# eps696/aphantasia

Hardware: NVIDIA H100
Metric: optimization steps/sec @1280x720 FFT, 200 samples, ViT-B/32 (higher is better)
Workload: dtype bf16

## Files before the change

aphantasia_b200/_lib.py:

```python
import ctypes as C
import os

_HERE = os.path.dirname(os.path.abspath(__file__))
LIB_PATH = os.path.join(_HERE, 'libaphb200.so')

_lib = None

c_f32p = C.c_void_p
_SIGS = {
    'aph_version': (C.c_int, []),
    'aph_last_error': (C.c_char_p, []),
    'aph_launch_count': (C.c_int64, []),
    'aph_fft_plan_create': (C.c_int, [C.POINTER(C.c_void_p), C.c_int, C.c_int]),
    'aph_fft_plan_destroy': (C.c_int, [C.c_void_p]),
    'aph_synth_fft_fwd': (C.c_int, [C.c_void_p, c_f32p, c_f32p, c_f32p, C.c_int, C.c_float, C.c_void_p, C.c_int,
                                    c_f32p, C.c_void_p, c_f32p, C.c_void_p]),
    'aph_synth_fft_bwd': (C.c_int, [C.c_void_p, c_f32p, c_f32p, c_f32p, C.c_void_p, c_f32p, C.c_float, C.c_void_p, C.c_int,
                                    c_f32p, C.c_void_p]),
    'aph_dwt_plan_create': (C.c_int, [C.POINTER(C.c_void_p), C.c_int, C.c_int, C.c_void_p, C.c_void_p, C.c_int]),
    'aph_dwt_plan_destroy': (C.c_int, [C.c_void_p]),
    'aph_dwt_plan_levels': (C.c_int, [C.c_void_p, C.POINTER(C.c_int), C.c_void_p, C.c_void_p]),
    'aph_synth_dwt_fwd': (C.c_int, [C.c_void_p, C.c_void_p, C.c_void_p, C.c_float, C.c_void_p, C.c_int, c_f32p, C.c_void_p, c_f32p, C.c_void_p]),
    'aph_synth_dwt_bwd': (C.c_int, [C.c_void_p, c_f32p, c_f32p, c_f32p, C.c_void_p, C.c_void_p, C.c_float, C.c_void_p, C.c_int, C.c_void_p, C.c_void_p]),
    'aph_pixel_fwd': (C.c_int, [c_f32p, C.c_int64, C.c_float, C.c_int, C.c_void_p, C.c_int, C.c_void_p, c_f32p, C.c_void_p]),
    'aph_pixel_bwd': (C.c_int, [c_f32p, c_f32p, c_f32p, C.c_void_p, C.c_int64, C.c_float, C.c_int, C.c_void_p, C.c_int, c_f32p, C.c_void_p]),
    'aph_valid_rgb_fwd': (C.c_int, [c_f32p, C.c_int64, C.c_void_p, c_f32p, C.c_void_p]),
    'aph_valid_rgb_bwd': (C.c_int, [c_f32p, c_f32p, C.c_int64, C.c_void_p, c_f32p, C.c_void_p]),
    'aph_sample_fwd': (C.c_int, [c_f32p, C.c_int, C.c_int, C.c_int, C.c_int, c_f32p, C.c_int, C.c_int, C.c_int, c_f32p, C.c_void_p]),
    'aph_sample_fwd_patches': (C.c_int, [c_f32p, C.c_int, C.c_int, C.c_int, C.c_int, c_f32p, C.c_int, C.c_int, C.c_int, c_f32p, C.c_void_p, C.c_int,
                                         C.POINTER(C.c_int), C.c_void_p]),
    'aph_sample_bwd': (C.c_int, [c_f32p, C.c_int, C.c_int, C.c_int, C.c_int, c_f32p, C.c_int, C.c_int, C.c_int, c_f32p, C.c_void_p]),
    'aph_sample_bwd_scaled': (C.c_int, [c_f32p, C.c_int, C.c_int, C.c_int, C.c_int, c_f32p, C.c_int, C.c_int, C.c_int, C.c_float, c_f32p, C.c_void_p]),
    'aph_rng_crop_tables': (C.c_int, [C.c_void_p, C.c_int64, C.c_void_p, C.POINTER(C.c_int32), C.c_void_p, C.c_void_p, C.c_void_p, C.c_int,
                                      C.c_int, C.c_int, C.c_int, C.c_int, C.c_int, C.c_int, C.c_float, C.c_int, C.c_void_p]),
    'aph_vit_create': (C.c_int, [C.POINTER(C.c_void_p), C.c_void_p]),
    'aph_vit_destroy': (C.c_int, [C.c_void_p]),
    'aph_vit_load_tensor': (C.c_int, [C.c_void_p, C.c_char_p, c_f32p, C.c_int64, C.c_void_p]),
    'aph_vit_finalize': (C.c_int, [C.c_void_p]),
    'aph_vit_fwd': (C.c_int, [C.c_void_p, c_f32p, C.c_int, c_f32p, C.c_int, C.c_void_p]),
    'aph_vit_patch_operand': (C.c_int, [C.c_void_p, C.c_int, C.POINTER(C.c_void_p), C.POINTER(C.c_int), C.POINTER(C.c_int)]),
    'aph_vit_fwd_prepatched': (C.c_int, [C.c_void_p, C.c_int, c_f32p, C.c_int, C.c_void_p]),
    'aph_vit_bwd': (C.c_int, [C.c_void_p, c_f32p, C.c_int, c_f32p, C.c_void_p]),
    'aph_vit_bytes': (C.c_int64, [C.c_void_p]),
    'aph_text_create': (C.c_int, [C.POINTER(C.c_void_p), C.c_void_p]),
    'aph_text_destroy': (C.c_int, [C.c_void_p]),
    'aph_text_load_tensor': (C.c_int, [C.c_void_p, C.c_char_p, c_f32p, C.c_int64, C.c_void_p]),
    'aph_text_finalize': (C.c_int, [C.c_void_p]),
    'aph_text_fwd': (C.c_int, [C.c_void_p, C.c_void_p, C.c_int, c_f32p, C.c_void_p]),
    'aph_text_bytes': (C.c_int64, [C.c_void_p]),
    'aph_gemm_bf16_tn': (C.c_int, [C.c_void_p, C.c_void_p, c_f32p, C.c_int, C.c_int, C.c_int, C.c_void_p]),
    'aph_gemm_epi_test': (C.c_int, [C.c_void_p, C.c_void_p, C.c_int, C.c_int, C.c_int, c_f32p, c_f32p, C.c_void_p, C.c_int, c_f32p, C.c_void_p, C.c_void_p,
                                    C.c_int, C.c_int, C.c_void_p]),
    'aph_gemm_variant_launches': (C.c_int64, [C.c_int, C.c_int]),
    'aph_prof_gemm': (C.c_int, [C.c_int, C.POINTER(C.c_double), C.POINTER(C.c_double), C.POINTER(C.c_int)]),
    'aph_sim_fwd': (C.c_int, [c_f32p, C.c_int, c_f32p, C.c_int, C.c_int, C.c_int, c_f32p, c_f32p, c_f32p, C.c_void_p]),
    'aph_derivat_fwd': (C.c_int, [c_f32p, C.c_int, C.c_int, C.c_int, C.c_void_p, c_f32p, C.c_void_p]),
    'aph_derivat_bwd': (C.c_int, [c_f32p, C.c_int, C.c_int, C.c_int, c_f32p, c_f32p, C.c_void_p]),
    'aph_head_fwd': (C.c_int, [c_f32p, C.c_int, C.c_int, c_f32p, c_f32p, c_f32p, C.c_void_p]),
    'aph_head_bwd': (C.c_int, [c_f32p, c_f32p, C.c_int, C.c_int, c_f32p, C.c_void_p]),
    'aph_synth_fft_bwd_adam': (C.c_int, [C.c_void_p, c_f32p, c_f32p, c_f32p, C.c_void_p, c_f32p, C.c_float, C.c_void_p, C.c_int,
                                         c_f32p, c_f32p, c_f32p, c_f32p, C.c_float, C.c_float, C.c_float, C.c_float, C.c_int, C.c_void_p]),
    'aph_allreduce_sym': (C.c_int, [C.c_uint64, C.c_void_p, C.c_uint64, C.c_int, C.c_int, C.c_int64, C.c_void_p, C.c_void_p]),
    'aph_adam_step': (C.c_int, [c_f32p, c_f32p, c_f32p, c_f32p, C.c_int64, C.c_float, C.c_float, C.c_float, C.c_float, C.c_int, C.c_void_p]),
}
EXPORTS = tuple(_SIGS)


class VitConfig(C.Structure):
    _fields_ = [(n, C.c_int32) for n in ('patch', 'width', 'layers', 'heads', 'out_dim', 'res', 'max_batch', 'reserved')]


class TextConfig(C.Structure):
    _fields_ = [(n, C.c_int32) for n in ('width', 'layers', 'heads', 'out_dim', 'context', 'vocab', 'max_batch', 'reserved')]


def lib():
    global _lib
    if _lib is None:
        if not os.path.isfile(LIB_PATH):
            raise RuntimeError('aphantasia_b200: %s not built. Run `python -c "import __graft_entry__ as g; g.build()"` '
                               '(or `make -C aphantasia_b200/csrc`). There is no CPU fallback.' % LIB_PATH)
        l = C.CDLL(LIB_PATH)
        for name, (res, args) in _SIGS.items():
            f = getattr(l, name)
            f.restype, f.argtypes = res, args
        _lib = l
    return _lib


def check(rc, what):
    if rc != 0:
        raise RuntimeError('%s failed (rc=%d): %s' % (what, rc, lib().aph_last_error().decode('utf-8', 'replace')))


def stream_ptr():
    import torch
    return torch.cuda.current_stream().cuda_stream


def require_cuda(t, name):
    import torch
    if not (isinstance(t, torch.Tensor) and t.is_cuda):
        raise RuntimeError('aphantasia_b200: %s must be a CUDA tensor; this implementation has no CPU path' % name)
```

aphantasia_b200/csrc/tc_gemm.cuh:

```cuda
#pragma once
#include "aph_common.cuh"
#include <cuda.h>

namespace aph {

typedef __nv_bfloat16 bf16;

struct GemmEpi {
  const float* bias = nullptr;
  const float* resid = nullptr;
  const bf16* gelu_in = nullptr;
  float* out_f32 = nullptr;
  bf16* out_bf16 = nullptr;
  bf16* out_pre = nullptr;
  int act = 0;
  int unpatch_p = 0;
  int unpatch_g = 0;
};

struct GemmShape { int M, N, K; };

constexpr int GEMM_BM = 128;
constexpr int GEMM_BK = 64;
constexpr int GEMM_UK = 16;
constexpr int GEMM_THREADS = 3 * 128;

enum : int {
  EPI_F32 = 0,
  EPI_BF16 = 1,
  EPI_BIAS_BF16 = 2,
  EPI_BIAS_GELU = 3,
  EPI_BIAS_RESID = 4,
  EPI_GELUGRAD_BF16 = 5,
  EPI_UNPATCH = 6,
  EPI_KINDS = 7
};

__device__ __forceinline__ uint32_t smem_u32(const void* p) { return (uint32_t)__cvta_generic_to_shared(p); }

__device__ __forceinline__ void mbar_init(uint64_t* bar, uint32_t count) {
  asm volatile("mbarrier.init.shared::cta.b64 [%0], %1;" ::"r"(smem_u32(bar)), "r"(count));
}
__device__ __forceinline__ void mbar_expect_tx(uint64_t* bar, uint32_t bytes) {
  asm volatile("mbarrier.arrive.expect_tx.shared::cta.b64 _, [%0], %1;" ::"r"(smem_u32(bar)), "r"(bytes) : "memory");
}
__device__ __forceinline__ void mbar_arrive(uint64_t* bar) {
  asm volatile("mbarrier.arrive.shared::cta.b64 _, [%0];" ::"r"(smem_u32(bar)) : "memory");
}
__device__ __forceinline__ void mbar_wait(uint64_t* bar, uint32_t parity) {
  uint32_t done;
  do {
    asm volatile(
        "{\n\t.reg .pred p;\n\t"
        "mbarrier.try_wait.parity.shared::cta.b64 p, [%1], %2;\n\t"
        "selp.u32 %0, 1, 0, p;\n\t}"
        : "=r"(done) : "r"(smem_u32(bar)), "r"(parity) : "memory");
  } while (!done);
}
__device__ __forceinline__ void fence_barrier_init() { asm volatile("fence.mbarrier_init.release.cluster;" ::: "memory"); }

__device__ __forceinline__ void tma_prefetch_desc(const CUtensorMap* m) {
  asm volatile("prefetch.tensormap [%0];" ::"l"(reinterpret_cast<uint64_t>(m)) : "memory");
}
__device__ __forceinline__ void tma_load_2d(void* dst, const CUtensorMap* m, uint64_t* bar, int x, int y) {
  asm volatile("cp.async.bulk.tensor.2d.shared::cluster.global.mbarrier::complete_tx::bytes [%0], [%1, {%3, %4}], [%2];"
               ::"r"(smem_u32(dst)), "l"(reinterpret_cast<uint64_t>(m)), "r"(smem_u32(bar)), "r"(x), "r"(y) : "memory");
}
__device__ __forceinline__ void tma_load_3d(uint32_t dst_saddr, const CUtensorMap* m, uint64_t* bar, int x, int y, int z) {
  asm volatile("cp.async.bulk.tensor.3d.shared::cluster.global.mbarrier::complete_tx::bytes [%0], [%1, {%3, %4, %5}], [%2];"
               ::"r"(dst_saddr), "l"(reinterpret_cast<uint64_t>(m)), "r"(smem_u32(bar)), "r"(x), "r"(y), "r"(z) : "memory");
}
__device__ __forceinline__ void tma_load_2d_hint(void* dst, const CUtensorMap* m, uint64_t* bar, int x, int y, uint64_t policy) {
  asm volatile("cp.async.bulk.tensor.2d.shared::cluster.global.mbarrier::complete_tx::bytes.L2::cache_hint [%0], [%1, {%3, %4}], [%2], %5;"
               ::"r"(smem_u32(dst)), "l"(reinterpret_cast<uint64_t>(m)), "r"(smem_u32(bar)), "r"(x), "r"(y), "l"(policy) : "memory");
}
__device__ __forceinline__ uint64_t l2_policy_evict_last() {
  uint64_t p;
  asm volatile("createpolicy.fractional.L2::evict_last.b64 %0, 1.0;" : "=l"(p));
  return p;
}

__device__ __forceinline__ uint64_t make_smem_desc(uint32_t saddr) {
  uint64_t d = 0;
  d |= (uint64_t)((saddr & 0x3FFFF) >> 4);
  d |= (uint64_t)1 << 16;
  d |= (uint64_t)(1024 >> 4) << 32;
  d |= (uint64_t)1 << 62;
  return d;
}
__device__ __forceinline__ void wgmma_fence() { asm volatile("wgmma.fence.sync.aligned;" ::: "memory"); }
__device__ __forceinline__ void wgmma_commit() { asm volatile("wgmma.commit_group.sync.aligned;" ::: "memory"); }
template <int N> __device__ __forceinline__ void wgmma_wait() { asm volatile("wgmma.wait_group.sync.aligned %0;" ::"n"(N) : "memory"); }
template <int R> __device__ __forceinline__ void setmaxnreg_inc() { asm volatile("setmaxnreg.inc.sync.aligned.u32 %0;" ::"n"(R)); }
template <int R> __device__ __forceinline__ void setmaxnreg_dec() { asm volatile("setmaxnreg.dec.sync.aligned.u32 %0;" ::"n"(R)); }

template <int BN> struct Wgmma;
#define APH_WG_REGS8(o) "+f"(d[o]), "+f"(d[o + 1]), "+f"(d[o + 2]), "+f"(d[o + 3]), "+f"(d[o + 4]), "+f"(d[o + 5]), "+f"(d[o + 6]), "+f"(d[o + 7])
template <> struct Wgmma<128> {
  static __device__ __forceinline__ void mma(float (&d)[64], uint64_t da, uint64_t db, int acc) {
    asm volatile(
        "{\n\t.reg .pred p;\n\tsetp.ne.b32 p, %66, 0;\n\t"
        "wgmma.mma_async.sync.aligned.m64n128k16.f32.bf16.bf16 "
        "{%0, %1, %2, %3, %4, %5, %6, %7, %8, %9, %10, %11, %12, %13, %14, %15, %16, %17, %18, %19, %20, %21, %22, %23, "
        "%24, %25, %26, %27, %28, %29, %30, %31, %32, %33, %34, %35, %36, %37, %38, %39, %40, %41, %42, %43, %44, %45, %46, %47, "
        "%48, %49, %50, %51, %52, %53, %54, %55, %56, %57, %58, %59, %60, %61, %62, %63}, %64, %65, p, 1, 1, 0, 0;\n\t}"
        : APH_WG_REGS8(0), APH_WG_REGS8(8), APH_WG_REGS8(16), APH_WG_REGS8(24), APH_WG_REGS8(32), APH_WG_REGS8(40), APH_WG_REGS8(48), APH_WG_REGS8(56)
        : "l"(da), "l"(db), "r"(acc));
  }
};
template <> struct Wgmma<256> {
  static __device__ __forceinline__ void mma(float (&d)[128], uint64_t da, uint64_t db, int acc) {
    asm volatile(
        "{\n\t.reg .pred p;\n\tsetp.ne.b32 p, %130, 0;\n\t"
        "wgmma.mma_async.sync.aligned.m64n256k16.f32.bf16.bf16 "
        "{%0, %1, %2, %3, %4, %5, %6, %7, %8, %9, %10, %11, %12, %13, %14, %15, %16, %17, %18, %19, %20, %21, %22, %23, "
        "%24, %25, %26, %27, %28, %29, %30, %31, %32, %33, %34, %35, %36, %37, %38, %39, %40, %41, %42, %43, %44, %45, %46, %47, "
        "%48, %49, %50, %51, %52, %53, %54, %55, %56, %57, %58, %59, %60, %61, %62, %63, %64, %65, %66, %67, %68, %69, %70, %71, "
        "%72, %73, %74, %75, %76, %77, %78, %79, %80, %81, %82, %83, %84, %85, %86, %87, %88, %89, %90, %91, %92, %93, %94, %95, "
        "%96, %97, %98, %99, %100, %101, %102, %103, %104, %105, %106, %107, %108, %109, %110, %111, %112, %113, %114, %115, "
        "%116, %117, %118, %119, %120, %121, %122, %123, %124, %125, %126, %127}, %128, %129, p, 1, 1, 0, 0;\n\t}"
        : APH_WG_REGS8(0), APH_WG_REGS8(8), APH_WG_REGS8(16), APH_WG_REGS8(24), APH_WG_REGS8(32), APH_WG_REGS8(40), APH_WG_REGS8(48), APH_WG_REGS8(56),
          APH_WG_REGS8(64), APH_WG_REGS8(72), APH_WG_REGS8(80), APH_WG_REGS8(88), APH_WG_REGS8(96), APH_WG_REGS8(104), APH_WG_REGS8(112), APH_WG_REGS8(120)
        : "l"(da), "l"(db), "r"(acc));
  }
};
#undef APH_WG_REGS8

__device__ __forceinline__ float sigmoid1702(float x) {
  float t;
  asm("tanh.approx.f32 %0, %1;" : "=f"(t) : "f"(0.851f * x));
  return fmaf(0.5f, t, 0.5f);
}
__device__ __forceinline__ float quickgelu(float x) { return x * sigmoid1702(x); }
__device__ __forceinline__ float quickgelu_grad(float x) {
  const float s = sigmoid1702(x);
  return s * (1.f + 1.702f * x * (1.f - s));
}
__device__ __forceinline__ uint32_t pack_bf16(float lo, float hi) {
  __nv_bfloat162 v = __floats2bfloat162_rn(lo, hi);
  return *reinterpret_cast<uint32_t*>(&v);
}

template <int BN>
struct GemmCfg {
  static constexpr int A_BYTES = GEMM_BM * GEMM_BK * 2;
  static constexpr int B_BYTES = BN * GEMM_BK * 2;
  static constexpr int STAGE_BYTES = A_BYTES + B_BYTES;
  static constexpr int STAGES = (BN == 256) ? 4 : 6;
  static constexpr int BAR_OFFSET = STAGES * STAGE_BYTES;
  static constexpr int SMEM = BAR_OFFSET + 2 * STAGES * 8 + 1024;
};

__device__ __forceinline__ void consumer_bar_sync(int id) { asm volatile("bar.sync %0, 256;" ::"r"(id) : "memory"); }
__device__ __forceinline__ void consumer_bar_arrive(int id) { asm volatile("bar.arrive %0, 256;" ::"r"(id) : "memory"); }

template <int EPI>
constexpr bool epi_bf16_out() { return EPI == EPI_BF16 || EPI == EPI_BIAS_BF16 || EPI == EPI_BIAS_GELU || EPI == EPI_GELUGRAD_BF16; }

template <int EPI>
__device__ __forceinline__ void epi_store2(const GemmEpi& epi, int N, int row, int col, float v0, float v1, float2 bb) {
  const size_t off = (size_t)row * N + col;
  if (EPI == EPI_F32) {
    *reinterpret_cast<float2*>(epi.out_f32 + off) = make_float2(v0, v1);
  } else if (EPI == EPI_BIAS_RESID) {
    const float2 r = __ldg(reinterpret_cast<const float2*>(epi.resid + off));
    *reinterpret_cast<float2*>(epi.out_f32 + off) = make_float2(v0 + bb.x + r.x, v1 + bb.y + r.y);
  } else {
    const int p = epi.unpatch_p, g = epi.unpatch_g, R = p * g;
    const int ch = col / (p * p), rem = col - ch * p * p, py = rem / p, px = rem - py * p;
    const int s = row / (g * g), pr = row - s * g * g, gy = pr / g, gx = pr - gy * g;
    *reinterpret_cast<float2*>(epi.out_f32 + (((size_t)s * 3 + ch) * R + gy * p + py) * R + gx * p + px) = make_float2(v0, v1);
  }
}

__device__ __forceinline__ void st_global_16(void* p, const uint32_t (&w)[4]) {
  asm volatile("st.global.v4.b32 [%0], {%1, %2, %3, %4};" ::"l"(p), "r"(w[0]), "r"(w[1]), "r"(w[2]), "r"(w[3]) : "memory");
}

__device__ __forceinline__ void quad_transpose(uint32_t (&w)[4], int q) {
  const bool b0 = q & 1, b1 = q & 2;
#pragma unroll
  for (int p = 0; p < 2; ++p) {
    const uint32_t r = __shfl_xor_sync(0xffffffffu, b0 ? w[2 * p] : w[2 * p + 1], 1);
    if (b0) w[2 * p] = r; else w[2 * p + 1] = r;
  }
#pragma unroll
  for (int p = 0; p < 2; ++p) {
    const uint32_t r = __shfl_xor_sync(0xffffffffu, b1 ? w[p] : w[p + 2], 2);
    if (b1) w[p] = r; else w[p + 2] = r;
  }
}

template <int EPI>
__device__ __forceinline__ void epi_store_bf16x32(const GemmEpi& epi, int N, int row, bool valid, int col0, int q, const float* v,
                                                  const float2* bb) {
  const size_t off = (size_t)row * N + col0 + 8 * q;
  uint32_t w[4], w2[4];
  if constexpr (EPI == EPI_GELUGRAD_BF16) {
    uint4 g = make_uint4(0u, 0u, 0u, 0u);
    if (valid) g = __ldg(reinterpret_cast<const uint4*>(epi.gelu_in + off));
    w2[0] = g.x; w2[1] = g.y; w2[2] = g.z; w2[3] = g.w;
    quad_transpose(w2, q);
  }
#pragma unroll
  for (int t = 0; t < 4; ++t) {
    float v0 = v[2 * t], v1 = v[2 * t + 1];
    if (EPI == EPI_BF16) {
      w[t] = pack_bf16(v0, v1);
    } else if (EPI == EPI_BIAS_BF16) {
      w[t] = pack_bf16(v0 + bb[t].x, v1 + bb[t].y);
    } else if (EPI == EPI_BIAS_GELU) {
      v0 += bb[t].x; v1 += bb[t].y;
      w2[t] = pack_bf16(v0, v1);
      w[t] = pack_bf16(quickgelu(v0), quickgelu(v1));
    } else {
      const float2 h = __bfloat1622float2(*reinterpret_cast<const __nv_bfloat162*>(&w2[t]));
      w[t] = pack_bf16(v0 * quickgelu_grad(h.x), v1 * quickgelu_grad(h.y));
    }
  }
  quad_transpose(w, q);
  if (valid) st_global_16(epi.out_bf16 + off, w);
  if constexpr (EPI == EPI_BIAS_GELU) {
    quad_transpose(w2, q);
    if (valid) st_global_16(epi.out_pre + off, w2);
  }
}

template <int BN, bool PINGPONG, int EPI>
__global__ void __launch_bounds__(GEMM_THREADS, 1)
k_gemm_bf16_tn(const __grid_constant__ CUtensorMap map_a, const __grid_constant__ CUtensorMap map_b, GemmShape shp, GemmEpi epi) {
  static_assert(BN == 128 || !PINGPONG, "the ping-pong schedule runs 128 x 128 tiles");
  using L = GemmCfg<BN>;
  constexpr int STAGES = L::STAGES;
  constexpr int MMAS = PINGPONG ? 2 : 1;
  constexpr bool HAS_BIAS = (EPI == EPI_BIAS_BF16 || EPI == EPI_BIAS_GELU || EPI == EPI_BIAS_RESID);
  pdl_trigger();
  extern __shared__ uint8_t smem_raw[];
  uint8_t* smem = reinterpret_cast<uint8_t*>((reinterpret_cast<uintptr_t>(smem_raw) + 1023) & ~(uintptr_t)1023);
  uint64_t* full_bar = reinterpret_cast<uint64_t*>(smem + L::BAR_OFFSET);
  uint64_t* empty_bar = full_bar + STAGES;

  const int wg = threadIdx.x >> 7, tid = threadIdx.x & 127;
  const int m_tiles = (shp.M + GEMM_BM - 1) / GEMM_BM, n_tiles = shp.N / BN;
  const int num_tiles = m_tiles * n_tiles, k_blocks = shp.K / GEMM_BK;

  if (threadIdx.x == 0) {
    tma_prefetch_desc(&map_a); tma_prefetch_desc(&map_b);
    for (int i = 0; i < STAGES; ++i) { mbar_init(&full_bar[i], 1); mbar_init(&empty_bar[i], PINGPONG ? 1 : 2); }
    fence_barrier_init();
  }
  __syncthreads();
  pdl_wait();

  if (wg == 0) {
    setmaxnreg_dec<40>();
    if (tid == 0) {
      const uint64_t pol_b = l2_policy_evict_last();
      uint32_t it = 0;
      for (int tile = blockIdx.x; tile < num_tiles; tile += gridDim.x) {
        const int m_blk = tile / n_tiles, n_blk = tile - m_blk * n_tiles;
        for (int kb = 0; kb < k_blocks; ++kb, ++it) {
          const uint32_t s = it % STAGES, ph = (it / STAGES) & 1;
          mbar_wait(&empty_bar[s], ph ^ 1);
          uint8_t* sa = smem + s * L::STAGE_BYTES;
          mbar_expect_tx(&full_bar[s], L::STAGE_BYTES);
          tma_load_2d(sa, &map_a, &full_bar[s], kb * GEMM_BK, m_blk * GEMM_BM);
          tma_load_2d_hint(sa + L::A_BYTES, &map_b, &full_bar[s], kb * GEMM_BK, n_blk * BN, pol_b);
        }
      }
    }
  } else {
    setmaxnreg_inc<232>();
    const int c = wg - 1, warp = tid >> 5, lane = tid & 31;
    const int row_in_tile = (PINGPONG ? 0 : 64 * c) + 16 * warp + (lane >> 2), col_in_tile = 2 * (lane & 3);
    uint32_t it = PINGPONG ? c * k_blocks : 0;
    const int tile_step = (PINGPONG ? 2 : 1) * gridDim.x;
    for (int tile = blockIdx.x + (PINGPONG ? c * gridDim.x : 0); tile / n_tiles * GEMM_BM < shp.M; tile += tile_step) {
      if (PINGPONG && tile != (int)blockIdx.x) consumer_bar_sync(1 + c);
      float d[MMAS][BN / 2];
#pragma unroll
      for (int h = 0; h < MMAS; ++h)
#pragma unroll
        for (int r = 0; r < BN / 2; ++r) d[h][r] = 0.f;
      for (int kb = 0; kb < k_blocks; ++kb, ++it) {
        const uint32_t s = it % STAGES, ph = (it / STAGES) & 1;
        mbar_wait(&full_bar[s], ph);
        const uint64_t ds = make_smem_desc(smem_u32(smem + s * L::STAGE_BYTES));
        wgmma_fence();
#pragma unroll
        for (int k = 0; k < GEMM_BK / GEMM_UK; ++k)
#pragma unroll
          for (int h = 0; h < MMAS; ++h)
            Wgmma<BN>::mma(d[h], ds + (uint64_t)((PINGPONG ? h : c) * 512 + 2 * k), ds + (uint64_t)(L::A_BYTES / 16 + 2 * k), (kb | k) != 0);
        wgmma_commit();
        wgmma_wait<1>();
        if (kb > 0 && tid == 0) mbar_arrive(&empty_bar[(it - 1) % STAGES]);
      }
      if (PINGPONG && (tile + (int)gridDim.x) / n_tiles * GEMM_BM < shp.M) consumer_bar_arrive(1 + (c ^ 1));
      wgmma_wait<0>();
      if (tid == 0) mbar_arrive(&empty_bar[(it - 1) % STAGES]);
      if (PINGPONG) it += k_blocks;
      const int m_blk = tile / n_tiles, n_blk = tile - m_blk * n_tiles;
#pragma unroll
      for (int h = 0; h < MMAS; ++h) {
        const int row0 = m_blk * GEMM_BM + 64 * h + row_in_tile, row1 = row0 + 8;
        if constexpr (epi_bf16_out<EPI>()) {
#pragma unroll
          for (int j0 = 0; j0 < BN / 8; j0 += 4) {
            const int col0 = n_blk * BN + 8 * j0;
            float2 bb[4];
            float v0[8], v1[8];
#pragma unroll
            for (int t = 0; t < 4; ++t) {
              bb[t] = HAS_BIAS ? __ldg(reinterpret_cast<const float2*>(epi.bias + col0 + 8 * t + col_in_tile)) : make_float2(0.f, 0.f);
              v0[2 * t] = d[h][4 * (j0 + t)]; v0[2 * t + 1] = d[h][4 * (j0 + t) + 1];
              v1[2 * t] = d[h][4 * (j0 + t) + 2]; v1[2 * t + 1] = d[h][4 * (j0 + t) + 3];
            }
            epi_store_bf16x32<EPI>(epi, shp.N, row0, row0 < shp.M, col0, lane & 3, v0, bb);
            epi_store_bf16x32<EPI>(epi, shp.N, row1, row1 < shp.M, col0, lane & 3, v1, bb);
          }
        } else {
#pragma unroll
          for (int j = 0; j < BN / 8; ++j) {
            const int col = n_blk * BN + 8 * j + col_in_tile;
            const float2 bb = HAS_BIAS ? __ldg(reinterpret_cast<const float2*>(epi.bias + col)) : make_float2(0.f, 0.f);
            if (row0 < shp.M) epi_store2<EPI>(epi, shp.N, row0, col, d[h][4 * j], d[h][4 * j + 1], bb);
            if (row1 < shp.M) epi_store2<EPI>(epi, shp.N, row1, col, d[h][4 * j + 2], d[h][4 * j + 3], bb);
          }
        }
      }
    }
  }
}

int make_tmap_bf16(CUtensorMap* out, const void* base, int rows, int K, int box_rows);
int make_tmap_bf16_tokens(CUtensorMap* out, const void* base, int cols, int T, int S, int box_rows);
int launch_gemm(const void* A, const void* B, GemmShape shp, const GemmEpi& epi, cudaStream_t st);

}
```

aphantasia_b200/csrc/vit.cu:

```cuda
#include "vit_ops.cuh"
#include "vit_attn_tc.cuh"
#include <stdlib.h>
#include <string>
#include <vector>
#include <map>
#include <string.h>

namespace aph {

struct LayerW {
  float *ln1_w = nullptr, *ln1_b = nullptr, *ln2_w = nullptr, *ln2_b = nullptr;
  float *b_qkv = nullptr, *b_o = nullptr, *b_fc = nullptr, *b_proj = nullptr;
  bf16 *w_qkv = nullptr, *w_qkv_t = nullptr;
  bf16 *w_o = nullptr, *w_o_t = nullptr;
  bf16 *w_fc = nullptr, *w_fc_t = nullptr;
  bf16 *w_proj = nullptr, *w_proj_t = nullptr;
};

struct VitImpl {
  aph_vit_config cfg;
  int g, T, D, Kp;
  int64_t bytes = 0;
  std::vector<void*> allocs;
  bf16 *w_conv = nullptr, *w_conv_t = nullptr;
  float *cls = nullptr, *pos = nullptr, *lnpre_w = nullptr, *lnpre_b = nullptr, *lnpost_w = nullptr, *lnpost_b = nullptr;
  bf16 *w_out = nullptr, *w_out_t = nullptr;
  std::vector<LayerW> L;
  std::map<std::string, bool> loaded;
  bool finalized = false;
  bf16* patches = nullptr;
  float* tok = nullptr;
  float* e = nullptr;
  std::vector<float*> xs;
  bf16* ln_out = nullptr;
  std::vector<bf16*> qkv;
  bf16* attn_out = nullptr;
  std::vector<bf16*> h_pre;
  bf16* h_act = nullptr;
  float *st_mean = nullptr, *st_rstd = nullptr;
  bf16* cls_ln = nullptr;
  float* emb_int = nullptr;
  bf16* d_emb = nullptr;
  float* d_cls = nullptr;
  float* dx = nullptr;
  bf16* dx_bf = nullptr;
  bf16* dh = nullptr;
  bf16* d_ln = nullptr;
  bf16* d_attn = nullptr;
  bf16* d_qkv = nullptr;
  bf16* d_tok = nullptr;
  int last_S = -1;
  struct GraphEntry { const void* in; const void* out; int S; int flag; cudaGraphExec_t exec; unsigned long long stamp; int nodes; };
  std::vector<GraphEntry> fwd_graphs, bwd_graphs;
  std::map<int, int> warm_fwd, warm_bwd;
  unsigned long long stamp = 0;
  int graph_misses = 0;
};

bool gemm_profiling_on();

static bool graphs_enabled() {
  static int v = -1;
  if (v < 0) { const char* e = getenv("APH_VIT_GRAPH"); v = (e && e[0] == '0') ? 0 : 1; }
  return v == 1 && !gemm_profiling_on();
}

template <typename Body>
static int run_cached(std::vector<VitImpl::GraphEntry>& cache, std::map<int, int>& warm, unsigned long long& stamp, int& misses,
                      const void* in, const void* out, int S, int flag, cudaStream_t& st, Body body) {
  if (!graphs_enabled() || misses > 6) return body();
  for (auto& g : cache)
    if (g.in == in && g.out == out && g.S == S && g.flag == flag) {
      g.stamp = ++stamp;
      misses = 0;
      APH_CUDA_OK(cudaGraphLaunch(g.exec, st));
      count_launch(g.nodes);
      return 0;
    }
  if (!warm[S]) { warm[S] = 1; return body(); }
  static cudaStream_t cap = nullptr;
  if (!cap) APH_CUDA_OK(cudaStreamCreateWithFlags(&cap, cudaStreamNonBlocking));
  cudaStream_t user = st;
  st = cap;
  if (cudaStreamBeginCapture(cap, cudaStreamCaptureModeThreadLocal) != cudaSuccess) { cudaGetLastError(); st = user; return body(); }
  const int rc = body();
  cudaGraph_t graph = nullptr;
  const cudaError_t ce = cudaStreamEndCapture(cap, &graph);
  st = user;
  if (rc != 0 || ce != cudaSuccess || graph == nullptr) {
    if (graph) cudaGraphDestroy(graph);
    cudaGetLastError();
    if (rc != 0) return rc;
    return body();
  }
  size_t nodes = 0;
  cudaGraphGetNodes(graph, nullptr, &nodes);
  g_launches.fetch_sub((long long)nodes, std::memory_order_relaxed);
  cudaGraphExec_t exec = nullptr;
  if (cudaGraphInstantiate(&exec, graph, 0) != cudaSuccess) { cudaGraphDestroy(graph); cudaGetLastError(); return body(); }
  cudaGraphDestroy(graph);
  if (cache.size() >= 4) {
    size_t lru = 0;
    for (size_t i = 1; i < cache.size(); ++i) if (cache[i].stamp < cache[lru].stamp) lru = i;
    cudaGraphExecDestroy(cache[lru].exec);
    cache.erase(cache.begin() + lru);
  }
  ++misses;
  cache.push_back({in, out, S, flag, exec, ++stamp, (int)nodes});
  APH_CUDA_OK(cudaGraphLaunch(exec, st));
  count_launch((int)nodes);
  return 0;
}

template <typename Tp>
static int dev_alloc(VitImpl* v, Tp** p, size_t count) {
  void* q = nullptr;
  APH_CUDA_OK(cudaMalloc(&q, count * sizeof(Tp)));
  v->allocs.push_back(q);
  v->bytes += (int64_t)(count * sizeof(Tp));
  *p = reinterpret_cast<Tp*>(q);
  return 0;
}

__global__ void __launch_bounds__(256) k_pack_weight(const float* __restrict__ in, bf16* __restrict__ out, int rows, int cols, int transpose) {
  const size_t n = (size_t)rows * cols;
  for (size_t i = blockIdx.x * (size_t)blockDim.x + threadIdx.x; i < n; i += (size_t)gridDim.x * blockDim.x) {
    const int r = (int)(i / cols), c = (int)(i - (size_t)r * cols);
    const bf16 v = __float2bfloat16_rn(in[i]);
    if (transpose) out[(size_t)c * rows + r] = v; else out[i] = v;
  }
}

int pack(const float* src, bf16* dst, int rows, int cols, int transpose, cudaStream_t st) {
  const size_t n = (size_t)rows * cols;
  const int blocks = (int)std::min<size_t>((n + 255) / 256, (size_t)num_sms() * 16);
  k_pack_weight<<<blocks, 256, 0, st>>>(src, dst, rows, cols, transpose);
  APH_LAUNCH_OK();
  return 0;
}

int copy_f32(const float* src, float* dst, size_t n, cudaStream_t st) {
  APH_CUDA_OK(cudaMemcpyAsync(dst, src, n * sizeof(float), cudaMemcpyDeviceToDevice, st));
  return 0;
}

static inline int rows_grid(int rows) { return (rows * 32 + 255) / 256; }

static bool attn_simt() {
  static int v = -1;
  if (v < 0) { const char* e = getenv("APH_ATTN_SIMT"); v = (e && e[0] == '1') ? 1 : 0; }
  return v == 1;
}

}

using namespace aph;

extern "C" int aph_vit_create(aph_vit** out, const aph_vit_config* cfg) {
  APH_REQUIRE(out && cfg, "aph_vit_create: null argument");
  APH_REQUIRE(cfg->width % 128 == 0 && (cfg->width / 128 == 1 || cfg->width / 128 == 2 || cfg->width / 128 == 6 || cfg->width / 128 == 8),
              "aph_vit_create: width %d unsupported (128, 256, 768, 1024)", cfg->width);
  APH_REQUIRE(cfg->heads * 64 == cfg->width, "aph_vit_create: head dim must be 64 (width %d, heads %d)", cfg->width, cfg->heads);
  APH_REQUIRE(cfg->res % cfg->patch == 0 && cfg->patch % 8 == 0, "aph_vit_create: res %d / patch %d", cfg->res, cfg->patch);
  APH_REQUIRE(cfg->out_dim % 128 == 0 && cfg->max_batch > 0 && cfg->layers > 0, "aph_vit_create: out_dim %d must be a multiple of 128", cfg->out_dim);
  VitImpl* v = new VitImpl();
  v->cfg = *cfg;
  v->g = cfg->res / cfg->patch; v->T = v->g * v->g + 1; v->D = cfg->width; v->Kp = 3 * cfg->patch * cfg->patch;
  APH_REQUIRE(v->T <= 256 && v->Kp % 128 == 0, "aph_vit_create: T=%d (max 256) Kp=%d", v->T, v->Kp);
  const int D = v->D, T = v->T, S = cfg->max_batch, Ly = cfg->layers, O = cfg->out_dim;
  const size_t M = (size_t)S * T, Mp = (size_t)S * v->g * v->g;
  int e = 0;
  e |= dev_alloc(v, &v->w_conv, (size_t)D * v->Kp); e |= dev_alloc(v, &v->w_conv_t, (size_t)D * v->Kp);
  e |= dev_alloc(v, &v->cls, D); e |= dev_alloc(v, &v->pos, (size_t)T * D);
  e |= dev_alloc(v, &v->lnpre_w, D); e |= dev_alloc(v, &v->lnpre_b, D); e |= dev_alloc(v, &v->lnpost_w, D); e |= dev_alloc(v, &v->lnpost_b, D);
  e |= dev_alloc(v, &v->w_out, (size_t)D * O); e |= dev_alloc(v, &v->w_out_t, (size_t)D * O);
  v->L.resize(Ly);
  for (auto& l : v->L) {
    e |= dev_alloc(v, &l.ln1_w, D); e |= dev_alloc(v, &l.ln1_b, D); e |= dev_alloc(v, &l.ln2_w, D); e |= dev_alloc(v, &l.ln2_b, D);
    e |= dev_alloc(v, &l.b_qkv, 3 * D); e |= dev_alloc(v, &l.b_o, D); e |= dev_alloc(v, &l.b_fc, 4 * D); e |= dev_alloc(v, &l.b_proj, D);
    e |= dev_alloc(v, &l.w_qkv, (size_t)3 * D * D); e |= dev_alloc(v, &l.w_qkv_t, (size_t)3 * D * D);
    e |= dev_alloc(v, &l.w_o, (size_t)D * D); e |= dev_alloc(v, &l.w_o_t, (size_t)D * D);
    e |= dev_alloc(v, &l.w_fc, (size_t)4 * D * D); e |= dev_alloc(v, &l.w_fc_t, (size_t)4 * D * D);
    e |= dev_alloc(v, &l.w_proj, (size_t)4 * D * D); e |= dev_alloc(v, &l.w_proj_t, (size_t)4 * D * D);
  }
  e |= dev_alloc(v, &v->patches, Mp * v->Kp); e |= dev_alloc(v, &v->tok, Mp * D); e |= dev_alloc(v, &v->e, M * D);
  v->xs.resize(2 * Ly + 1); for (auto& x : v->xs) e |= dev_alloc(v, &x, M * D);
  e |= dev_alloc(v, &v->ln_out, M * D); e |= dev_alloc(v, &v->attn_out, M * D); e |= dev_alloc(v, &v->h_act, M * 4 * D);
  v->qkv.resize(Ly); v->h_pre.resize(Ly);
  for (int i = 0; i < Ly; ++i) { e |= dev_alloc(v, &v->qkv[i], M * 3 * D); e |= dev_alloc(v, &v->h_pre[i], M * 4 * D); }
  e |= dev_alloc(v, &v->st_mean, (size_t)(2 * Ly + 2) * M); e |= dev_alloc(v, &v->st_rstd, (size_t)(2 * Ly + 2) * M);
  e |= dev_alloc(v, &v->cls_ln, (size_t)S * D); e |= dev_alloc(v, &v->emb_int, (size_t)S * O);
  e |= dev_alloc(v, &v->d_emb, (size_t)S * O); e |= dev_alloc(v, &v->d_cls, (size_t)S * D);
  e |= dev_alloc(v, &v->dx, M * D); e |= dev_alloc(v, &v->dx_bf, M * D); e |= dev_alloc(v, &v->dh, M * 4 * D);
  e |= dev_alloc(v, &v->d_ln, M * D); e |= dev_alloc(v, &v->d_attn, M * D); e |= dev_alloc(v, &v->d_qkv, M * 3 * D);
  e |= dev_alloc(v, &v->d_tok, Mp * D);
  if (e) { aph_vit_destroy(reinterpret_cast<aph_vit*>(v)); return 1; }
  APH_CUDA_OK(cudaFuncSetAttribute(k_attn_fwd, cudaFuncAttributeMaxDynamicSharedMemorySize, (int)attn_fwd_smem(T)));
  APH_CUDA_OK(cudaFuncSetAttribute(k_attn_bwd, cudaFuncAttributeMaxDynamicSharedMemorySize, (int)attn_bwd_smem(T)));
  *out = reinterpret_cast<aph_vit*>(v);
  return 0;
}

extern "C" int aph_vit_destroy(aph_vit* vit) {
  if (!vit) return 0;
  VitImpl* v = reinterpret_cast<VitImpl*>(vit);
  for (auto& g : v->fwd_graphs) cudaGraphExecDestroy(g.exec);
  for (auto& g : v->bwd_graphs) cudaGraphExecDestroy(g.exec);
  for (void* p : v->allocs) cudaFree(p);
  delete v;
  return 0;
}

extern "C" int64_t aph_vit_bytes(const aph_vit* vit) { return vit ? reinterpret_cast<const VitImpl*>(vit)->bytes : 0; }

extern "C" int aph_vit_load_tensor(aph_vit* vit, const char* key, const float* data, int64_t numel, void* stream) {
  APH_REQUIRE(vit && key && data, "aph_vit_load_tensor: null argument");
  VitImpl* v = reinterpret_cast<VitImpl*>(vit);
  cudaStream_t st = (cudaStream_t)stream;
  const int D = v->D, O = v->cfg.out_dim;
  std::string k(key);
  if (k.rfind("visual.", 0) == 0) k = k.substr(7);
  auto need = [&](int64_t n) -> int { APH_REQUIRE(numel == n, "aph_vit_load_tensor(%s): expected %lld elements, got %lld", key, (long long)n, (long long)numel); return 0; };
  int e = 0;
  if (k == "conv1.weight") { if ((e = need((int64_t)D * v->Kp))) return e; e = pack(data, v->w_conv, D, v->Kp, 0, st) | pack(data, v->w_conv_t, D, v->Kp, 1, st); }
  else if (k == "class_embedding") { if ((e = need(D))) return e; e = copy_f32(data, v->cls, D, st); }
  else if (k == "positional_embedding") { if ((e = need((int64_t)v->T * D))) return e; e = copy_f32(data, v->pos, (size_t)v->T * D, st); }
  else if (k == "ln_pre.weight") { if ((e = need(D))) return e; e = copy_f32(data, v->lnpre_w, D, st); }
  else if (k == "ln_pre.bias") { if ((e = need(D))) return e; e = copy_f32(data, v->lnpre_b, D, st); }
  else if (k == "ln_post.weight") { if ((e = need(D))) return e; e = copy_f32(data, v->lnpost_w, D, st); }
  else if (k == "ln_post.bias") { if ((e = need(D))) return e; e = copy_f32(data, v->lnpost_b, D, st); }
  else if (k == "proj") {
    if ((e = need((int64_t)D * O))) return e;
    e = pack(data, v->w_out, D, O, 1, st) | pack(data, v->w_out_t, D, O, 0, st);
  } else if (k.rfind("transformer.resblocks.", 0) == 0) {
    const char* rest = k.c_str() + strlen("transformer.resblocks.");
    char* endp = nullptr;
    const long li = strtol(rest, &endp, 10);
    APH_REQUIRE(endp && *endp == '.' && li >= 0 && li < v->cfg.layers, "aph_vit_load_tensor: bad layer index in %s", key);
    LayerW& l = v->L[li];
    const std::string f(endp + 1);
    if (f == "ln_1.weight") { if ((e = need(D))) return e; e = copy_f32(data, l.ln1_w, D, st); }
    else if (f == "ln_1.bias") { if ((e = need(D))) return e; e = copy_f32(data, l.ln1_b, D, st); }
    else if (f == "ln_2.weight") { if ((e = need(D))) return e; e = copy_f32(data, l.ln2_w, D, st); }
    else if (f == "ln_2.bias") { if ((e = need(D))) return e; e = copy_f32(data, l.ln2_b, D, st); }
    else if (f == "attn.in_proj_weight") { if ((e = need((int64_t)3 * D * D))) return e; e = pack(data, l.w_qkv, 3 * D, D, 0, st) | pack(data, l.w_qkv_t, 3 * D, D, 1, st); }
    else if (f == "attn.in_proj_bias") { if ((e = need(3 * D))) return e; e = copy_f32(data, l.b_qkv, 3 * D, st); }
    else if (f == "attn.out_proj.weight") { if ((e = need((int64_t)D * D))) return e; e = pack(data, l.w_o, D, D, 0, st) | pack(data, l.w_o_t, D, D, 1, st); }
    else if (f == "attn.out_proj.bias") { if ((e = need(D))) return e; e = copy_f32(data, l.b_o, D, st); }
    else if (f == "mlp.c_fc.weight") { if ((e = need((int64_t)4 * D * D))) return e; e = pack(data, l.w_fc, 4 * D, D, 0, st) | pack(data, l.w_fc_t, 4 * D, D, 1, st); }
    else if (f == "mlp.c_fc.bias") { if ((e = need(4 * D))) return e; e = copy_f32(data, l.b_fc, 4 * D, st); }
    else if (f == "mlp.c_proj.weight") { if ((e = need((int64_t)4 * D * D))) return e; e = pack(data, l.w_proj, D, 4 * D, 0, st) | pack(data, l.w_proj_t, D, 4 * D, 1, st); }
    else if (f == "mlp.c_proj.bias") { if ((e = need(D))) return e; e = copy_f32(data, l.b_proj, D, st); }
    else { set_error("aph_vit_load_tensor: unknown tensor %s", key); return 2; }
  } else { set_error("aph_vit_load_tensor: unknown tensor %s", key); return 2; }
  if (e) return e;
  v->loaded[k] = true;
  return 0;
}

extern "C" int aph_vit_finalize(aph_vit* vit) {
  APH_REQUIRE(vit, "aph_vit_finalize: null handle");
  VitImpl* v = reinterpret_cast<VitImpl*>(vit);
  std::vector<std::string> want = {"conv1.weight", "class_embedding", "positional_embedding", "ln_pre.weight", "ln_pre.bias",
                                   "ln_post.weight", "ln_post.bias", "proj"};
  const char* per[] = {"ln_1.weight", "ln_1.bias", "ln_2.weight", "ln_2.bias", "attn.in_proj_weight", "attn.in_proj_bias",
                       "attn.out_proj.weight", "attn.out_proj.bias", "mlp.c_fc.weight", "mlp.c_fc.bias", "mlp.c_proj.weight", "mlp.c_proj.bias"};
  for (int i = 0; i < v->cfg.layers; ++i)
    for (const char* p : per) want.push_back("transformer.resblocks." + std::to_string(i) + "." + p);
  for (const auto& w : want) APH_REQUIRE(v->loaded.count(w), "aph_vit_finalize: tensor visual.%s was never loaded", w.c_str());
  v->finalized = true;
  return 0;
}

static int vit_fwd_impl(aph_vit* vit, const float* images, int S, float* emb, int save_for_bwd, void* stream);

extern "C" int aph_vit_fwd(aph_vit* vit, const float* images, int S, float* emb, int save_for_bwd, void* stream) {
  APH_REQUIRE(vit && images && emb, "aph_vit_fwd: null argument");
  return vit_fwd_impl(vit, images, S, emb, save_for_bwd, stream);
}

extern "C" int aph_vit_patch_operand(aph_vit* vit, int S, void** patches_bf16, int* patch, int* grid) {
  APH_REQUIRE(vit && patches_bf16 && patch && grid, "aph_vit_patch_operand: null argument");
  VitImpl* v = reinterpret_cast<VitImpl*>(vit);
  APH_REQUIRE(v->finalized, "aph_vit_patch_operand: weights not finalized");
  APH_REQUIRE(S > 0 && S <= v->cfg.max_batch, "aph_vit_patch_operand: S=%d outside (0, max_batch=%d]", S, v->cfg.max_batch);
  *patches_bf16 = v->patches; *patch = v->cfg.patch; *grid = v->g;
  return 0;
}

extern "C" int aph_vit_fwd_prepatched(aph_vit* vit, int S, float* emb, int save_for_bwd, void* stream) {
  APH_REQUIRE(vit && emb, "aph_vit_fwd_prepatched: null argument");
  return vit_fwd_impl(vit, nullptr, S, emb, save_for_bwd, stream);
}

static int vit_fwd_impl(aph_vit* vit, const float* images, int S, float* emb, int save_for_bwd, void* stream) {
  VitImpl* v = reinterpret_cast<VitImpl*>(vit);
  APH_REQUIRE(v->finalized, "aph_vit_fwd: weights not finalized");
  APH_REQUIRE(S > 0 && S <= v->cfg.max_batch, "aph_vit_fwd: S=%d outside (0, max_batch=%d]", S, v->cfg.max_batch);
  cudaStream_t st = (cudaStream_t)stream;
  if (images) {
    const int g = v->g, Mp = S * g * g;
    const size_t n8 = (size_t)Mp * v->Kp / 8;
    APH_CUDA_OK(launch_k(k_patchify, dim3((unsigned)std::min<size_t>((n8 + 255) / 256, (size_t)num_sms() * 16)), dim3(256), (size_t)0, st, 1, images, v->patches, S, v->cfg.patch, g));
    APH_LAUNCH_OK();
  }
  const int rc = run_cached(v->fwd_graphs, v->warm_fwd, v->stamp, v->graph_misses, nullptr, nullptr, S, save_for_bwd, st, [&]() -> int {
  const int D = v->D, T = v->T, g = v->g, Ly = v->cfg.layers, O = v->cfg.out_dim, H = v->cfg.heads;
  const int M = S * T, Mp = S * g * g;
  const size_t Mmax = (size_t)v->cfg.max_batch * T;
  int e;
  {
    GemmEpi ep; ep.out_f32 = v->tok;
    if ((e = launch_gemm(v->patches, v->w_conv, GemmShape{Mp, D, v->Kp}, ep, st))) return e;
    NCH_DISPATCH(D, APH_CUDA_OK(launch_k(k_embed_lnpre<NCH>, dim3(rows_grid(M)), dim3(256), (size_t)0, st, 1, v->tok, v->cls, v->pos, v->lnpre_w, v->lnpre_b, v->e, v->xs[0],
                                                                      v->st_mean, v->st_rstd, S, T, D)));
    APH_LAUNCH_OK();
  }
  for (int l = 0; l < Ly; ++l) {
    const LayerW& w = v->L[l];
    float* x_in = v->xs[2 * l]; float* x_mid = v->xs[2 * l + 1]; float* x_out = v->xs[2 * l + 2];
    float* mean1 = v->st_mean + (size_t)(1 + 2 * l) * Mmax; float* rstd1 = v->st_rstd + (size_t)(1 + 2 * l) * Mmax;
    float* mean2 = mean1 + Mmax; float* rstd2 = rstd1 + Mmax;
    NCH_DISPATCH(D, APH_CUDA_OK(launch_k(k_ln_fwd<NCH>, dim3(rows_grid(M)), dim3(256), (size_t)0, st, 1, x_in, (size_t)D, w.ln1_w, w.ln1_b, v->ln_out, mean1, rstd1, M, D)));
    APH_LAUNCH_OK();
    { GemmEpi ep; ep.bias = w.b_qkv; ep.out_bf16 = v->qkv[l];
      if ((e = launch_gemm(v->ln_out, w.w_qkv, GemmShape{M, 3 * D, D}, ep, st))) return e; }
    if (attn_simt()) { k_attn_fwd<<<S * H, 256, attn_fwd_smem(T), st>>>(v->qkv[l], v->attn_out, T, D, H); APH_LAUNCH_OK(); }
    else if ((e = attn_dispatch(true, v->qkv[l], nullptr, v->attn_out, S, T, D, H, st))) return e;
    { GemmEpi ep; ep.bias = w.b_o; ep.resid = x_in; ep.out_f32 = x_mid;
      if ((e = launch_gemm(v->attn_out, w.w_o, GemmShape{M, D, D}, ep, st))) return e; }
    NCH_DISPATCH(D, APH_CUDA_OK(launch_k(k_ln_fwd<NCH>, dim3(rows_grid(M)), dim3(256), (size_t)0, st, 1, x_mid, (size_t)D, w.ln2_w, w.ln2_b, v->ln_out, mean2, rstd2, M, D)));
    APH_LAUNCH_OK();
    { GemmEpi ep; ep.bias = w.b_fc; ep.out_pre = v->h_pre[l]; ep.act = 1; ep.out_bf16 = v->h_act;
      if ((e = launch_gemm(v->ln_out, w.w_fc, GemmShape{M, 4 * D, D}, ep, st))) return e; }
    { GemmEpi ep; ep.bias = w.b_proj; ep.resid = x_mid; ep.out_f32 = x_out;
      if ((e = launch_gemm(v->h_act, w.w_proj, GemmShape{M, D, 4 * D}, ep, st))) return e; }
  }
  {
    float* meanp = v->st_mean + (size_t)(2 * Ly + 1) * Mmax; float* rstdp = v->st_rstd + (size_t)(2 * Ly + 1) * Mmax;
    NCH_DISPATCH(D, APH_CUDA_OK(launch_k(k_ln_fwd<NCH>, dim3(rows_grid(S)), dim3(256), (size_t)0, st, 1, v->xs[2 * Ly], (size_t)T * D, v->lnpost_w, v->lnpost_b, v->cls_ln,
                                                                 meanp, rstdp, S, D)));
    APH_LAUNCH_OK();
    GemmEpi ep; ep.out_f32 = v->emb_int;
    if ((e = launch_gemm(v->cls_ln, v->w_out, GemmShape{S, O, D}, ep, st))) return e;
  }
  return 0;
  });
  if (rc) return rc;
  APH_CUDA_OK(cudaMemcpyAsync(emb, v->emb_int, (size_t)S * v->cfg.out_dim * sizeof(float), cudaMemcpyDeviceToDevice, st));
  v->last_S = save_for_bwd ? S : -1;
  return 0;
}

extern "C" int aph_vit_bwd(aph_vit* vit, const float* grad_emb, int S, float* grad_images, void* stream) {
  APH_REQUIRE(vit && grad_emb && grad_images, "aph_vit_bwd: null argument");
  VitImpl* v = reinterpret_cast<VitImpl*>(vit);
  APH_REQUIRE(v->last_S == S, "aph_vit_bwd: no saved forward for S=%d (last saved S=%d)", S, v->last_S);
  cudaStream_t st = (cudaStream_t)stream;
  {
    const size_t n = (size_t)S * v->cfg.out_dim;
    APH_CUDA_OK(launch_k(k_f32_to_bf16, dim3((int)std::min<size_t>((n + 255) / 256, (size_t)num_sms() * 8)), dim3(256), (size_t)0, st, 1, grad_emb, v->d_emb, n));
    APH_LAUNCH_OK();
  }
  const int rc = run_cached(v->bwd_graphs, v->warm_bwd, v->stamp, v->graph_misses, nullptr, nullptr, S, 0, st, [&]() -> int {
  const int D = v->D, T = v->T, Ly = v->cfg.layers, O = v->cfg.out_dim, H = v->cfg.heads;
  const int M = S * T;
  const size_t Mmax = (size_t)v->cfg.max_batch * T;
  int e;
  {
    GemmEpi ep; ep.out_f32 = v->d_cls;
    if ((e = launch_gemm(v->d_emb, v->w_out_t, GemmShape{S, D, O}, ep, st))) return e;
    APH_CUDA_OK(cudaMemsetAsync(v->dx, 0, (size_t)M * D * sizeof(float), st));
    APH_CUDA_OK(cudaMemsetAsync(v->dx_bf, 0, (size_t)M * D * sizeof(bf16), st));
    float* meanp = v->st_mean + (size_t)(2 * Ly + 1) * Mmax; float* rstdp = v->st_rstd + (size_t)(2 * Ly + 1) * Mmax;
    NCH_DISPATCH(D, APH_CUDA_OK(launch_k(k_ln_bwd<NCH>, dim3(rows_grid(S)), dim3(256), (size_t)0, st, 1, v->d_cls, v->xs[2 * Ly], meanp, rstdp, v->lnpost_w, v->dx, v->dx_bf,
                                                                 S, T, D, 1, 0)));
    APH_LAUNCH_OK();
  }
  for (int l = Ly - 1; l >= 0; --l) {
    const LayerW& w = v->L[l];
    float* x_in = v->xs[2 * l]; float* x_mid = v->xs[2 * l + 1];
    float* mean1 = v->st_mean + (size_t)(1 + 2 * l) * Mmax; float* rstd1 = v->st_rstd + (size_t)(1 + 2 * l) * Mmax;
    float* mean2 = mean1 + Mmax; float* rstd2 = rstd1 + Mmax;
    { GemmEpi ep; ep.gelu_in = v->h_pre[l]; ep.out_bf16 = v->dh;
      if ((e = launch_gemm(v->dx_bf, w.w_proj_t, GemmShape{M, 4 * D, D}, ep, st))) return e; }
    { GemmEpi ep; ep.out_bf16 = v->d_ln;
      if ((e = launch_gemm(v->dh, w.w_fc_t, GemmShape{M, D, 4 * D}, ep, st))) return e; }
    NCH_DISPATCH(D, APH_CUDA_OK(launch_k(k_ln_bwd<NCH, bf16>, dim3(rows_grid(M)), dim3(256), (size_t)0, st, 1, v->d_ln, x_mid, mean2, rstd2, w.ln2_w, v->dx, v->dx_bf, M, T, D, 0, 1)));
    APH_LAUNCH_OK();
    { GemmEpi ep; ep.out_bf16 = v->d_attn;
      if ((e = launch_gemm(v->dx_bf, w.w_o_t, GemmShape{M, D, D}, ep, st))) return e; }
    if (attn_simt()) { k_attn_bwd<<<S * H, 256, attn_bwd_smem(T), st>>>(v->qkv[l], v->d_attn, v->d_qkv, T, D, H); APH_LAUNCH_OK(); }
    else if ((e = attn_dispatch(false, v->qkv[l], v->d_attn, v->d_qkv, S, T, D, H, st))) return e;
    { GemmEpi ep; ep.out_bf16 = v->d_ln;
      if ((e = launch_gemm(v->d_qkv, w.w_qkv_t, GemmShape{M, D, 3 * D}, ep, st))) return e; }
    NCH_DISPATCH(D, APH_CUDA_OK(launch_k(k_ln_bwd<NCH, bf16>, dim3(rows_grid(M)), dim3(256), (size_t)0, st, 1, v->d_ln, x_in, mean1, rstd1, w.ln1_w, v->dx, v->dx_bf, M, T, D, 0, 1)));
    APH_LAUNCH_OK();
  }
  NCH_DISPATCH(D, APH_CUDA_OK(launch_k(k_ln_bwd<NCH>, dim3(rows_grid(M)), dim3(256), (size_t)0, st, 1, v->dx, v->e, v->st_mean, v->st_rstd, v->lnpre_w, nullptr, v->d_tok, M, T, D, 2, 0)));
  APH_LAUNCH_OK();
  return 0;
  });
  if (rc) return rc;
  { const int g = v->g, Mp = S * g * g;
    GemmEpi ep; ep.out_f32 = grad_images; ep.unpatch_p = v->cfg.patch; ep.unpatch_g = g;
    if (int e = launch_gemm(v->d_tok, v->w_conv_t, GemmShape{Mp, v->Kp, v->D}, ep, st)) return e; }
  return 0;
}
```

aphantasia_b200/csrc/vit_gemm.cu:

```cuda
#include "tc_gemm.cuh"
#include <atomic>
#include <mutex>
#include <vector>
#include <utility>

namespace aph {

typedef CUresult (*EncodeTiledFn)(CUtensorMap*, CUtensorMapDataType, cuuint32_t, void*, const cuuint64_t*, const cuuint64_t*,
                                  const cuuint32_t*, const cuuint32_t*, CUtensorMapInterleave, CUtensorMapSwizzle,
                                  CUtensorMapL2promotion, CUtensorMapFloatOOBfill);

static EncodeTiledFn get_encode() {
  static EncodeTiledFn fn = nullptr;
  static std::once_flag once;
  std::call_once(once, [] {
    void* p = nullptr;
    cudaDriverEntryPointQueryResult q;
    if (cudaGetDriverEntryPoint("cuTensorMapEncodeTiled", &p, cudaEnableDefault, &q) == cudaSuccess && q == cudaDriverEntryPointSuccess)
      fn = reinterpret_cast<EncodeTiledFn>(p);
  });
  return fn;
}

int make_tmap_bf16(CUtensorMap* out, const void* base, int rows, int K, int box_rows) {
  EncodeTiledFn enc = get_encode();
  APH_REQUIRE(enc != nullptr, "cuTensorMapEncodeTiled not available from the driver");
  APH_REQUIRE((reinterpret_cast<uintptr_t>(base) & 15) == 0 && K % 8 == 0, "tensor map: base/stride not 16-byte aligned");
  const cuuint64_t gdim[2] = {(cuuint64_t)K, (cuuint64_t)rows};
  const cuuint64_t gstride[1] = {(cuuint64_t)K * 2};
  const cuuint32_t box[2] = {(cuuint32_t)GEMM_BK, (cuuint32_t)box_rows};
  const cuuint32_t estr[2] = {1, 1};
  const CUresult r = enc(out, CU_TENSOR_MAP_DATA_TYPE_BFLOAT16, 2, const_cast<void*>(base), gdim, gstride, box, estr,
                         CU_TENSOR_MAP_INTERLEAVE_NONE, CU_TENSOR_MAP_SWIZZLE_128B, CU_TENSOR_MAP_L2_PROMOTION_L2_256B,
                         CU_TENSOR_MAP_FLOAT_OOB_FILL_NONE);
  APH_REQUIRE(r == CUDA_SUCCESS, "cuTensorMapEncodeTiled failed: CUresult %d (rows=%d K=%d box_rows=%d)", (int)r, rows, K, box_rows);
  return 0;
}

int make_tmap_bf16_tokens(CUtensorMap* out, const void* base, int cols, int T, int S, int box_rows) {
  EncodeTiledFn enc = get_encode();
  APH_REQUIRE(enc != nullptr, "cuTensorMapEncodeTiled not available from the driver");
  APH_REQUIRE((reinterpret_cast<uintptr_t>(base) & 15) == 0 && cols % 8 == 0, "tensor map: base/stride not 16-byte aligned");
  const cuuint64_t gdim[3] = {(cuuint64_t)cols, (cuuint64_t)T, (cuuint64_t)S};
  const cuuint64_t gstride[2] = {(cuuint64_t)cols * 2, (cuuint64_t)T * cols * 2};
  const cuuint32_t box[3] = {64u, (cuuint32_t)box_rows, 1u};
  const cuuint32_t estr[3] = {1, 1, 1};
  const CUresult r = enc(out, CU_TENSOR_MAP_DATA_TYPE_BFLOAT16, 3, const_cast<void*>(base), gdim, gstride, box, estr,
                         CU_TENSOR_MAP_INTERLEAVE_NONE, CU_TENSOR_MAP_SWIZZLE_128B, CU_TENSOR_MAP_L2_PROMOTION_L2_256B,
                         CU_TENSOR_MAP_FLOAT_OOB_FILL_NONE);
  APH_REQUIRE(r == CUDA_SUCCESS, "cuTensorMapEncodeTiled (tokens) failed: CUresult %d (cols=%d T=%d S=%d box_rows=%d)", (int)r, cols, T, S, box_rows);
  return 0;
}

static bool g_prof = false;
bool gemm_profiling_on() { return g_prof; }
static std::vector<std::pair<cudaEvent_t, cudaEvent_t>> g_prof_ev;
static std::vector<double> g_prof_flops;

static std::atomic<long long> g_variant_launches[2][EPI_KINDS];

template <int BN, bool PINGPONG, int EPI>
static int launch_cfg(const void* A, const void* B, GemmShape shp, const GemmEpi& epi, cudaStream_t st) {
  using L = GemmCfg<BN>;
  static_assert(L::SMEM <= 227 * 1024, "GEMM shared-memory budget");
  g_variant_launches[(PINGPONG || BN == 256) ? 1 : 0][EPI].fetch_add(1, std::memory_order_relaxed);
  static bool configured = false;
  if (!configured) {
    APH_CUDA_OK(cudaFuncSetAttribute(k_gemm_bf16_tn<BN, PINGPONG, EPI>, cudaFuncAttributeMaxDynamicSharedMemorySize, L::SMEM));
    configured = true;
  }
  CUtensorMap ma, mb;
  if (int e = make_tmap_bf16(&ma, A, shp.M, shp.K, GEMM_BM)) return e;
  if (int e = make_tmap_bf16(&mb, B, shp.N, shp.K, BN)) return e;
  const int tiles = ((shp.M + GEMM_BM - 1) / GEMM_BM) * (shp.N / BN);
  const int grid = tiles < num_sms() ? tiles : num_sms();
  cudaEvent_t e0 = nullptr, e1 = nullptr;
  if (g_prof) { cudaEventCreate(&e0); cudaEventCreate(&e1); cudaEventRecord(e0, st); }
  APH_CUDA_OK(launch_k(k_gemm_bf16_tn<BN, PINGPONG, EPI>, dim3(grid), dim3(GEMM_THREADS), (size_t)L::SMEM, st, 1, ma, mb, shp, epi));
  APH_LAUNCH_OK();
  if (g_prof) { cudaEventRecord(e1, st); g_prof_ev.emplace_back(e0, e1); g_prof_flops.push_back(2.0 * shp.M * shp.N * shp.K); }
  return 0;
}

int launch_gemm(const void* A, const void* B, GemmShape shp, const GemmEpi& epi, cudaStream_t st) {
  APH_REQUIRE(A && B && shp.M > 0, "gemm: null operand or empty M");
  APH_REQUIRE(shp.K % GEMM_BK == 0 && shp.K > 0, "gemm: K=%d must be a positive multiple of %d", shp.K, GEMM_BK);
  APH_REQUIRE(shp.N % 128 == 0 && shp.N > 0, "gemm: N=%d must be a positive multiple of 128", shp.N);
  int kind = -1;
  const bool b = epi.bias, r = epi.resid, gi = epi.gelu_in, f = epi.out_f32, h = epi.out_bf16, pre = epi.out_pre, act = epi.act == 1, un = epi.unpatch_p > 0;
  if (un && f && !b && !r && !gi && !h && !pre && !act) kind = EPI_UNPATCH;
  else if (f && !h && !b && !r && !gi && !pre && !act) kind = EPI_F32;
  else if (h && !f && !b && !r && !gi && !pre && !act) kind = EPI_BF16;
  else if (h && !f && b && !r && !gi && !pre && !act) kind = EPI_BIAS_BF16;
  else if (h && !f && b && !r && !gi && pre && act) kind = EPI_BIAS_GELU;
  else if (f && !h && b && r && !gi && !pre && !act) kind = EPI_BIAS_RESID;
  else if (h && !f && !b && !r && gi && !pre && !act) kind = EPI_GELUGRAD_BF16;
  APH_REQUIRE(kind >= 0, "gemm: unsupported epilogue combination");
  const uintptr_t bf16_ptrs = reinterpret_cast<uintptr_t>(epi.out_bf16) | reinterpret_cast<uintptr_t>(epi.out_pre) | reinterpret_cast<uintptr_t>(epi.gelu_in);
  APH_REQUIRE((bf16_ptrs & 15) == 0, "gemm: bf16 epilogue operands must be 16-byte aligned (8 columns are stored per lane)");
  const int m_tiles = (shp.M + GEMM_BM - 1) / GEMM_BM;
  const bool pingpong = m_tiles * (shp.N / 128) >= 2 * num_sms() && shp.K <= 1024;
  const bool wide = !pingpong && shp.N % 256 == 0 && m_tiles * (shp.N / 256) >= num_sms();
#define APH_GEMM_CASE(K) case K: return pingpong ? launch_cfg<128, true, K>(A, B, shp, epi, st) \
                                                 : wide ? launch_cfg<256, false, K>(A, B, shp, epi, st) : launch_cfg<128, false, K>(A, B, shp, epi, st);
  switch (kind) {
    APH_GEMM_CASE(EPI_F32) APH_GEMM_CASE(EPI_BF16) APH_GEMM_CASE(EPI_BIAS_BF16) APH_GEMM_CASE(EPI_BIAS_GELU)
    APH_GEMM_CASE(EPI_BIAS_RESID) APH_GEMM_CASE(EPI_GELUGRAD_BF16) APH_GEMM_CASE(EPI_UNPATCH)
  }
#undef APH_GEMM_CASE
  return 2;
}

}

using namespace aph;

extern "C" int aph_gemm_bf16_tn(const void* A, const void* B, float* C, int M, int N, int K, void* stream) {
  APH_REQUIRE(C != nullptr, "aph_gemm_bf16_tn: null output");
  GemmEpi epi;
  epi.out_f32 = C;
  return launch_gemm(A, B, GemmShape{M, N, K}, epi, (cudaStream_t)stream);
}

extern "C" int aph_gemm_epi_test(const void* A, const void* B, int M, int N, int K, const float* bias, const float* resid,
                                 const void* gelu_in, int act, float* out_f32, void* out_bf16, void* out_pre,
                                 int unpatch_p, int unpatch_g, void* stream) {
  GemmEpi epi;
  epi.bias = bias; epi.resid = resid; epi.gelu_in = reinterpret_cast<const bf16*>(gelu_in); epi.act = act;
  epi.out_f32 = out_f32; epi.out_bf16 = reinterpret_cast<bf16*>(out_bf16); epi.out_pre = reinterpret_cast<bf16*>(out_pre);
  epi.unpatch_p = unpatch_p; epi.unpatch_g = unpatch_g;
  return launch_gemm(A, B, GemmShape{M, N, K}, epi, (cudaStream_t)stream);
}

extern "C" int64_t aph_gemm_variant_launches(int variant, int epi) {
  if (variant < 0 || variant > 1 || epi >= EPI_KINDS) return -1;
  long long n = 0;
  for (int k = 0; k < EPI_KINDS; ++k) if (epi < 0 || epi == k) n += g_variant_launches[variant][k].load();
  return (int64_t)n;
}

extern "C" int aph_prof_gemm(int enable, double* total_ms, double* total_flops, int* launches) {
  if (enable) { g_prof = true; g_prof_ev.clear(); g_prof_flops.clear(); return 0; }
  g_prof = false;
  double ms = 0., fl = 0.;
  for (size_t i = 0; i < g_prof_ev.size(); ++i) {
    APH_CUDA_OK(cudaEventSynchronize(g_prof_ev[i].second));
    float t = 0.f;
    APH_CUDA_OK(cudaEventElapsedTime(&t, g_prof_ev[i].first, g_prof_ev[i].second));
    ms += t; fl += g_prof_flops[i];
    cudaEventDestroy(g_prof_ev[i].first); cudaEventDestroy(g_prof_ev[i].second);
  }
  if (total_ms) *total_ms = ms;
  if (total_flops) *total_flops = fl;
  if (launches) *launches = (int)g_prof_ev.size();
  g_prof_ev.clear(); g_prof_flops.clear();
  return 0;
}
```

aphantasia_b200/csrc/vit_ops.cuh:

```cuda
#pragma once
#include "tc_gemm.cuh"

namespace aph {

#define NCH_DISPATCH(D, ...)                                                           \
  switch ((D) / 128) {                                                                 \
    case 1: { constexpr int NCH = 1; __VA_ARGS__; } break;                             \
    case 2: { constexpr int NCH = 2; __VA_ARGS__; } break;                             \
    case 4: { constexpr int NCH = 4; __VA_ARGS__; } break;                             \
    case 6: { constexpr int NCH = 6; __VA_ARGS__; } break;                             \
    case 8: { constexpr int NCH = 8; __VA_ARGS__; } break;                             \
    default: set_error("vit: unsupported width %d", (D)); return 2;                    \
  }

static __global__ void __launch_bounds__(256) k_patchify(const float* __restrict__ img, bf16* __restrict__ out, int S, int p, int g) {
  pdl_trigger(); pdl_wait();
  const int R = p * g, Kp = 3 * p * p;
  const size_t total = (size_t)S * g * g * Kp / 8;
  for (size_t idx = blockIdx.x * (size_t)blockDim.x + threadIdx.x; idx < total; idx += (size_t)gridDim.x * blockDim.x) {
    const size_t e = idx * 8;
    const int row = (int)(e / Kp), col = (int)(e - (size_t)row * Kp);
    const int s = row / (g * g), pr = row - s * g * g, gy = pr / g, gx = pr - gy * g;
    const int c = col / (p * p), rem = col - c * p * p, py = rem / p, px = rem - py * p;
    const float* src = img + (((size_t)s * 3 + c) * R + gy * p + py) * R + gx * p + px;
    const float4 a = __ldg(reinterpret_cast<const float4*>(src)), b = __ldg(reinterpret_cast<const float4*>(src) + 1);
    __nv_bfloat162 p0 = __floats2bfloat162_rn(a.x, a.y), p1 = __floats2bfloat162_rn(a.z, a.w);
    __nv_bfloat162 p2 = __floats2bfloat162_rn(b.x, b.y), p3 = __floats2bfloat162_rn(b.z, b.w);
    uint4 u; u.x = *reinterpret_cast<uint32_t*>(&p0); u.y = *reinterpret_cast<uint32_t*>(&p1);
    u.z = *reinterpret_cast<uint32_t*>(&p2); u.w = *reinterpret_cast<uint32_t*>(&p3);
    *reinterpret_cast<uint4*>(out + e) = u;
  }
}

static __global__ void __launch_bounds__(256) k_f32_to_bf16(const float* __restrict__ in, bf16* __restrict__ out, size_t n) {
  pdl_trigger(); pdl_wait();
  for (size_t i = blockIdx.x * (size_t)blockDim.x + threadIdx.x; i < n; i += (size_t)gridDim.x * blockDim.x)
    out[i] = __float2bfloat16_rn(in[i]);
}


struct RowStats { float mean, rstd; };

template <int N>
__device__ __forceinline__ RowStats row_stats(const float (&v)[N], int D) {
  float s = 0.f;
#pragma unroll
  for (int i = 0; i < N; ++i) s += v[i];
  const float mean = warp_sum(s) / (float)D;
  float q = 0.f;
#pragma unroll
  for (int i = 0; i < N; ++i) { const float d = v[i] - mean; q += d * d; }
  const float var = warp_sum(q) / (float)D;
  return {mean, rsqrtf(var + 1e-5f)};
}

template <int N>
__device__ __forceinline__ void load_row(const float* __restrict__ row, float (&v)[N], int lane) {
#pragma unroll
  for (int k = 0; k < N / 4; ++k) {
    const float4 a = *reinterpret_cast<const float4*>(row + (k * 32 + lane) * 4);
    v[4 * k] = a.x; v[4 * k + 1] = a.y; v[4 * k + 2] = a.z; v[4 * k + 3] = a.w;
  }
}
template <int N>
__device__ __forceinline__ void load_row(const bf16* __restrict__ row, float (&v)[N], int lane) {
#pragma unroll
  for (int k = 0; k < N / 4; ++k) {
    const uint2 u = *reinterpret_cast<const uint2*>(row + (k * 32 + lane) * 4);
    const float2 a = __bfloat1622float2(*reinterpret_cast<const __nv_bfloat162*>(&u.x)), b = __bfloat1622float2(*reinterpret_cast<const __nv_bfloat162*>(&u.y));
    v[4 * k] = a.x; v[4 * k + 1] = a.y; v[4 * k + 2] = b.x; v[4 * k + 3] = b.y;
  }
}
template <int N>
__device__ __forceinline__ void store_row_f32(float* __restrict__ row, const float (&v)[N], int lane) {
#pragma unroll
  for (int k = 0; k < N / 4; ++k)
    *reinterpret_cast<float4*>(row + (k * 32 + lane) * 4) = make_float4(v[4 * k], v[4 * k + 1], v[4 * k + 2], v[4 * k + 3]);
}
template <int N>
__device__ __forceinline__ void store_row_bf16(bf16* __restrict__ row, const float (&v)[N], int lane) {
#pragma unroll
  for (int k = 0; k < N / 4; ++k) {
    __nv_bfloat162 p0 = __floats2bfloat162_rn(v[4 * k], v[4 * k + 1]), p1 = __floats2bfloat162_rn(v[4 * k + 2], v[4 * k + 3]);
    uint2 u; u.x = *reinterpret_cast<uint32_t*>(&p0); u.y = *reinterpret_cast<uint32_t*>(&p1);
    *reinterpret_cast<uint2*>(row + (k * 32 + lane) * 4) = u;
  }
}

template <int NCH>
__global__ void __launch_bounds__(256) k_embed_lnpre(const float* __restrict__ tok, const float* __restrict__ cls,
                                                     const float* __restrict__ pos, const float* __restrict__ gamma,
                                                     const float* __restrict__ beta, float* __restrict__ e_out,
                                                     float* __restrict__ x0, float* __restrict__ mean_out, float* __restrict__ rstd_out,
                                                     int S, int T, int D) {
  pdl_trigger(); pdl_wait();
  const int row = (blockIdx.x * blockDim.x + threadIdx.x) >> 5, lane = threadIdx.x & 31;
  if (row >= S * T) return;
  const int s = row / T, t = row - s * T;
  constexpr int N = 4 * NCH;
  const float* src = (t == 0) ? cls : tok + ((size_t)s * (T - 1) + (t - 1)) * D;
  float v[N], pz[N];
  load_row(src, v, lane);
  load_row(pos + (size_t)t * D, pz, lane);
  #pragma unroll
  for (int i = 0; i < N; ++i) v[i] += pz[i];
  store_row_f32(e_out + (size_t)row * D, v, lane);
  const RowStats st = row_stats(v, D);
  float gm[N], bt[N];
  load_row(gamma, gm, lane); load_row(beta, bt, lane);
  #pragma unroll
  for (int i = 0; i < N; ++i) v[i] = (v[i] - st.mean) * st.rstd * gm[i] + bt[i];
  store_row_f32(x0 + (size_t)row * D, v, lane);
  if (lane == 0) { mean_out[row] = st.mean; rstd_out[row] = st.rstd; }
}

template <int NCH>
__global__ void __launch_bounds__(256) k_ln_fwd(const float* __restrict__ x, size_t in_stride, const float* __restrict__ gamma,
                                                const float* __restrict__ beta, bf16* __restrict__ y, float* __restrict__ mean_out,
                                                float* __restrict__ rstd_out, int rows, int D) {
  pdl_trigger(); pdl_wait();
  const int row = (blockIdx.x * blockDim.x + threadIdx.x) >> 5, lane = threadIdx.x & 31;
  if (row >= rows) return;
  constexpr int N = 4 * NCH;
  float v[N], gm[N], bt[N];
  load_row(x + (size_t)row * in_stride, v, lane);
  const RowStats st = row_stats(v, D);
  load_row(gamma, gm, lane); load_row(beta, bt, lane);
  #pragma unroll
  for (int i = 0; i < N; ++i) v[i] = (v[i] - st.mean) * st.rstd * gm[i] + bt[i];
  store_row_bf16(y + (size_t)row * D, v, lane);
  if (lane == 0) { mean_out[row] = st.mean; rstd_out[row] = st.rstd; }
}

template <int N>
__device__ __forceinline__ void ln_bwd_row(float (&v)[N], const float (&xv)[N], const float (&gm)[N], float mean, float rstd, int D) {
  float s1 = 0.f, s2 = 0.f;
#pragma unroll
  for (int i = 0; i < N; ++i) {
    const float xh = (xv[i] - mean) * rstd, dxh = v[i] * gm[i];
    s1 += dxh; s2 += dxh * xh;
  }
  s1 = warp_sum(s1) / (float)D; s2 = warp_sum(s2) / (float)D;
#pragma unroll
  for (int i = 0; i < N; ++i) {
    const float xh = (xv[i] - mean) * rstd, dxh = v[i] * gm[i];
    v[i] = rstd * (dxh - s1 - xh * s2);
  }
}

template <int NCH, typename DY = float>
__global__ void __launch_bounds__(256) k_ln_bwd(const DY* __restrict__ dy, const float* __restrict__ x, const float* __restrict__ mean,
                                                const float* __restrict__ rstd, const float* __restrict__ gamma,
                                                float* __restrict__ dx, bf16* __restrict__ dx_bf16, int rows, int T, int D,
                                                int mode, int accumulate) {
  pdl_trigger(); pdl_wait();
  const int r = (blockIdx.x * blockDim.x + threadIdx.x) >> 5, lane = threadIdx.x & 31;
  if (r >= rows) return;
  constexpr int N = 4 * NCH;
  const size_t row = (mode == 1) ? (size_t)r * T : (size_t)r;
  if (mode == 2 && (r % T) == 0) return;
  float v[N], xv[N], gm[N];
  load_row(dy + (size_t)r * D, v, lane);
  load_row(x + row * D, xv, lane);
  load_row(gamma, gm, lane);
  const int sidx = (mode == 1) ? r : (int)row;
  ln_bwd_row(v, xv, gm, mean[sidx], rstd[sidx], D);
  if (mode == 2) {
    const int s = r / T, t = r - s * T;
    store_row_bf16(dx_bf16 + ((size_t)s * (T - 1) + (t - 1)) * D, v, lane);
    return;
  }
  if (accumulate) {
    float a[N];
    load_row(dx + row * D, a, lane);
    #pragma unroll
  for (int i = 0; i < N; ++i) v[i] += a[i];
  }
  store_row_f32(dx + row * D, v, lane);
  store_row_bf16(dx_bf16 + row * D, v, lane);
}

constexpr int HD = 64;

static __global__ void __launch_bounds__(256) k_attn_fwd(const bf16* __restrict__ qkv, bf16* __restrict__ out, int T, int D, int heads) {
  extern __shared__ uint8_t sm_raw[];
  const int Tp = (T + 31) & ~31;
  const int Tq = Tp + 2;
  bf16* Kt = reinterpret_cast<bf16*>(sm_raw);
  bf16* V = Kt + HD * Tq;
  float* qs = reinterpret_cast<float*>(V + (size_t)Tp * HD);
  float* ps = qs + 8 * HD;
  const int s = blockIdx.x / heads, h = blockIdx.x - s * heads;
  const int warp = threadIdx.x >> 5, lane = threadIdx.x & 31;
  const size_t ld = (size_t)3 * D;
  const bf16* base = qkv + (size_t)s * T * ld + h * HD;
  for (int idx = threadIdx.x; idx < Tp * HD; idx += blockDim.x) {
    const int j = idx / HD, d = idx - j * HD;
    const bool ok = j < T;
    Kt[d * Tq + j] = ok ? base[(size_t)j * ld + D + d] : __float2bfloat16(0.f);
    if (ok) V[j * HD + d] = base[(size_t)j * ld + 2 * D + d];
  }
  __syncthreads();
  const int nj = Tp / 32;
  for (int i = warp; i < T; i += 8) {
    const __nv_bfloat162 q2 = *reinterpret_cast<const __nv_bfloat162*>(base + (size_t)i * ld + 2 * lane);
    const float2 qf = __bfloat1622float2(q2);
    qs[warp * HD + 2 * lane] = qf.x * 0.125f; qs[warp * HD + 2 * lane + 1] = qf.y * 0.125f;
    __syncwarp();
    float sc[8];
    float mx = -INFINITY;
    #pragma unroll
    for (int jj = 0; jj < 8; ++jj) if (jj < nj) {
      const int j = jj * 32 + lane;
      float a = 0.f;
#pragma unroll 16
      for (int d = 0; d < HD; ++d) a += qs[warp * HD + d] * __bfloat162float(Kt[d * Tq + j]);
      sc[jj] = (j < T) ? a : -INFINITY;
      mx = fmaxf(mx, sc[jj]);
    }
    mx = warp_max(mx);
    float sum = 0.f;
    #pragma unroll
    for (int jj = 0; jj < 8; ++jj) if (jj < nj) { const float p = __expf(sc[jj] - mx); sc[jj] = p; sum += p; }
    sum = warp_sum(sum);
    const float inv = 1.f / sum;
    #pragma unroll
    for (int jj = 0; jj < 8; ++jj) if (jj < nj) ps[warp * Tp + jj * 32 + lane] = sc[jj] * inv;
    __syncwarp();
    float o0 = 0.f, o1 = 0.f;
    for (int j = 0; j < T; ++j) {
      const float p = ps[warp * Tp + j];
      const float2 v = __bfloat1622float2(*reinterpret_cast<const __nv_bfloat162*>(V + j * HD + 2 * lane));
      o0 += p * v.x; o1 += p * v.y;
    }
    *reinterpret_cast<__nv_bfloat162*>(out + ((size_t)s * T + i) * D + h * HD + 2 * lane) = __floats2bfloat162_rn(o0, o1);
    __syncwarp();
  }
}

static __global__ void __launch_bounds__(256) k_attn_bwd(const bf16* __restrict__ qkv, const bf16* __restrict__ dout, bf16* __restrict__ dqkv,
                                                  int T, int D, int heads) {
  extern __shared__ uint8_t sm_raw[];
  const int Tp = (T + 31) & ~31;
  const int Tq = Tp + 2;
  bf16* Q = reinterpret_cast<bf16*>(sm_raw);
  bf16* K = Q + (size_t)Tp * HD;
  bf16* dO = K + (size_t)Tp * HD;
  bf16* Qt = dO + (size_t)Tp * HD;
  bf16* Kt = Qt + (size_t)Tq * HD;
  bf16* Vt = Kt + (size_t)Tq * HD;
  bf16* dOt = Vt + (size_t)Tq * HD;
  float* rmax = reinterpret_cast<float*>(dOt + (size_t)Tq * HD);
  float* rinv = rmax + Tp;
  float* rdel = rinv + Tp;
  float* va = rdel + Tp;
  float* vb = va + 8 * HD;
  float* s1 = vb + 8 * HD;
  float* s2 = s1 + 8 * Tp;
  const int s = blockIdx.x / heads, h = blockIdx.x - s * heads;
  const int warp = threadIdx.x >> 5, lane = threadIdx.x & 31;
  const size_t ld = (size_t)3 * D;
  const bf16* base = qkv + (size_t)s * T * ld + h * HD;
  const bf16* dbase = dout + (size_t)s * T * D + h * HD;
  const bf16 zero = __float2bfloat16(0.f);
  for (int idx = threadIdx.x; idx < Tp * HD; idx += blockDim.x) {
    const int j = idx / HD, d = idx - j * HD;
    const bool ok = j < T;
    const bf16 q = ok ? base[(size_t)j * ld + d] : zero, k = ok ? base[(size_t)j * ld + D + d] : zero;
    const bf16 v = ok ? base[(size_t)j * ld + 2 * D + d] : zero, g = ok ? dbase[(size_t)j * D + d] : zero;
    Q[j * HD + d] = q; Qt[d * Tq + j] = q; K[j * HD + d] = k; Kt[d * Tq + j] = k; Vt[d * Tq + j] = v;
    dO[j * HD + d] = g; dOt[d * Tq + j] = g;
  }
  __syncthreads();
  const int nj = Tp / 32;
  float* a = va + warp * HD; float* b = vb + warp * HD;
  float* p1 = s1 + warp * Tp; float* p2 = s2 + warp * Tp;
  for (int i = warp; i < T; i += 8) {
    {
      const float2 qf = __bfloat1622float2(*reinterpret_cast<const __nv_bfloat162*>(Q + i * HD + 2 * lane));
      const float2 gf = __bfloat1622float2(*reinterpret_cast<const __nv_bfloat162*>(dO + i * HD + 2 * lane));
      a[2 * lane] = qf.x * 0.125f; a[2 * lane + 1] = qf.y * 0.125f; b[2 * lane] = gf.x; b[2 * lane + 1] = gf.y;
    }
    __syncwarp();
    float sc[8], dp[8];
    float mx = -INFINITY;
    #pragma unroll
    for (int jj = 0; jj < 8; ++jj) if (jj < nj) {
      const int j = jj * 32 + lane;
      float x = 0.f, y = 0.f;
#pragma unroll 16
      for (int d = 0; d < HD; ++d) { x += a[d] * __bfloat162float(Kt[d * Tq + j]); y += b[d] * __bfloat162float(Vt[d * Tq + j]); }
      sc[jj] = (j < T) ? x : -INFINITY; dp[jj] = y;
      mx = fmaxf(mx, sc[jj]);
    }
    mx = warp_max(mx);
    float sum = 0.f;
    #pragma unroll
    for (int jj = 0; jj < 8; ++jj) if (jj < nj) { sc[jj] = __expf(sc[jj] - mx); sum += sc[jj]; }
    sum = warp_sum(sum);
    const float inv = 1.f / sum;
    float del = 0.f;
    #pragma unroll
    for (int jj = 0; jj < 8; ++jj) if (jj < nj) { sc[jj] *= inv; del += sc[jj] * dp[jj]; }
    del = warp_sum(del);
    #pragma unroll
    for (int jj = 0; jj < 8; ++jj) if (jj < nj) p2[jj * 32 + lane] = sc[jj] * (dp[jj] - del);
    if (lane == 0) { rmax[i] = mx; rinv[i] = inv; rdel[i] = del; }
    __syncwarp();
    float g0 = 0.f, g1 = 0.f;
    for (int j = 0; j < T; ++j) {
      const float ds = p2[j];
      const float2 kf = __bfloat1622float2(*reinterpret_cast<const __nv_bfloat162*>(K + j * HD + 2 * lane));
      g0 += ds * kf.x; g1 += ds * kf.y;
    }
    *reinterpret_cast<__nv_bfloat162*>(dqkv + ((size_t)s * T + i) * ld + h * HD + 2 * lane) = __floats2bfloat162_rn(g0 * 0.125f, g1 * 0.125f);
    __syncwarp();
  }
  __syncthreads();
  for (int j = warp; j < T; j += 8) {
    {
      const float2 kf = __bfloat1622float2(*reinterpret_cast<const __nv_bfloat162*>(K + j * HD + 2 * lane));
      a[2 * lane] = kf.x * 0.125f; a[2 * lane + 1] = kf.y * 0.125f;
      b[2 * lane] = __bfloat162float(Vt[(2 * lane) * Tq + j]); b[2 * lane + 1] = __bfloat162float(Vt[(2 * lane + 1) * Tq + j]);
    }
    __syncwarp();
    for (int ii = 0; ii < nj; ++ii) {
      const int i = ii * 32 + lane;
      float x = 0.f, y = 0.f;
#pragma unroll 16
      for (int d = 0; d < HD; ++d) { x += a[d] * __bfloat162float(Qt[d * Tq + i]); y += b[d] * __bfloat162float(dOt[d * Tq + i]); }
      float p = 0.f, ds = 0.f;
      if (i < T) { p = __expf(x - rmax[i]) * rinv[i]; ds = p * (y - rdel[i]); }
      p1[i] = p; p2[i] = ds;
    }
    __syncwarp();
    float k0 = 0.f, k1 = 0.f, v0 = 0.f, v1 = 0.f;
    for (int i = 0; i < T; ++i) {
      const float p = p1[i], ds = p2[i];
      const float2 qf = __bfloat1622float2(*reinterpret_cast<const __nv_bfloat162*>(Q + i * HD + 2 * lane));
      const float2 gf = __bfloat1622float2(*reinterpret_cast<const __nv_bfloat162*>(dO + i * HD + 2 * lane));
      k0 += ds * qf.x; k1 += ds * qf.y; v0 += p * gf.x; v1 += p * gf.y;
    }
    bf16* orow = dqkv + ((size_t)s * T + j) * ld + h * HD + 2 * lane;
    *reinterpret_cast<__nv_bfloat162*>(orow + D) = __floats2bfloat162_rn(k0 * 0.125f, k1 * 0.125f);
    *reinterpret_cast<__nv_bfloat162*>(orow + 2 * D) = __floats2bfloat162_rn(v0, v1);
    __syncwarp();
  }
}

inline size_t attn_fwd_smem(int T) { const int Tp = (T + 31) & ~31; return (size_t)(Tp + 2 + Tp) * HD * 2 + (8 * HD + 8 * Tp) * 4; }
inline size_t attn_bwd_smem(int T) { const int Tp = (T + 31) & ~31; return (size_t)(3 * Tp + 4 * (Tp + 2)) * HD * 2 + (3 * Tp + 16 * HD + 16 * Tp) * 4; }

}
```

include/aphb200.h:

```cpp
#ifndef APHB200_H_
#define APHB200_H_
#include <stddef.h>
#include <stdint.h>

#ifdef __cplusplus
extern "C" {
#endif

#define APH_ABI_VERSION 1

#define APH_CROP_PARAM_FLOATS 24
#define APH_F_OFFY   0
#define APH_F_OFFX   1
#define APH_F_CSIZE  2
#define APH_F_FLAGS  3
#define APH_F_PERSP  4
#define APH_F_ER_I   12
#define APH_F_ER_J   13
#define APH_F_ER_H   14
#define APH_F_ER_W   15
#define APH_F_ROT    16
#define APH_F_ANGLE  20
#define APH_FLAG_PERSP 1
#define APH_FLAG_ERASE 2
#define APH_FLAG_ROT   4

#define APH_TF_NONE      0
#define APH_TF_NORMALIZE 1
#define APH_TF_FAST      2

#define APH_SIM_COS 0
#define APH_SIM_MIX 1

int         aph_version(void);
const char* aph_last_error(void);

typedef struct aph_fft_plan aph_fft_plan;
int aph_fft_plan_create(aph_fft_plan** plan, int H, int W);
int aph_fft_plan_destroy(aph_fft_plan* plan);

int aph_synth_fft_fwd(aph_fft_plan* plan, const float* params, const float* scale,
                      const float* shift, int shift_mode, float contrast,
                      const float* colmat_host, int apply_sigmoid,
                      float* x_raw, double* stats, float* out, void* stream);
int aph_synth_fft_bwd(aph_fft_plan* plan, const float* grad_out, const float* out,
                      const float* x_raw, double* stats, const float* scale, float contrast,
                      const float* colmat_host, int apply_sigmoid,
                      float* grad_params, void* stream);

typedef struct aph_dwt_plan aph_dwt_plan;
int aph_dwt_plan_create(aph_dwt_plan** plan, int H, int W, const float* rec_lo_host, const float* rec_hi_host, int L);
int aph_dwt_plan_destroy(aph_dwt_plan* plan);
int aph_dwt_plan_levels(const aph_dwt_plan* plan, int* J, int* dims, int* out_hw);
int aph_synth_dwt_fwd(aph_dwt_plan* plan, const float* const* Ys, const float* scales_host, float contrast,
                      const float* colmat_host, int apply_sigmoid, float* x_raw, double* stats, float* out,
                      void* stream);
int aph_synth_dwt_bwd(aph_dwt_plan* plan, const float* grad_out, const float* out, const float* x_raw,
                      double* stats, const float* scales_host, float contrast, const float* colmat_host,
                      int apply_sigmoid, float* const* grad_Ys, void* stream);

int aph_pixel_fwd(const float* x, int64_t hw, float contrast, int fixcontrast, const float* colmat_host,
                  int apply_sigmoid, double* stats, float* out, void* stream);
int aph_pixel_bwd(const float* grad_out, const float* out, const float* x, double* stats, int64_t hw, float contrast,
                  int fixcontrast, const float* colmat_host, int apply_sigmoid, float* grad_x, void* stream);

int aph_valid_rgb_fwd(const float* img, int64_t hw, const float* colmat_host, float* out, void* stream);
int aph_valid_rgb_bwd(const float* grad_out, const float* out, int64_t hw, const float* colmat_host,
                      float* grad_img, void* stream);

int aph_sample_fwd(const float* canvas, int H, int W, int pad_top, int pad_left,
                   const float* table, int S, int size, int kind, float* out, void* stream);
int aph_sample_fwd_patches(const float* canvas, int H, int W, int pad_top, int pad_left,
                           const float* table, int S, int size, int kind, float* out,
                           void* patches_bf16, int patch, int* patches_written, void* stream);
int aph_sample_bwd(const float* grad_out, int H, int W, int pad_top, int pad_left,
                   const float* table, int S, int size, int kind, float* grad_canvas, void* stream);

int aph_sample_bwd_scaled(const float* grad_out, int H, int W, int pad_top, int pad_left,
                          const float* table, int S, int size, int kind, float gscale, float* grad_canvas, void* stream);

int aph_rng_crop_tables(uint8_t* torch_state, int64_t torch_state_bytes, uint32_t* np_key, int32_t* np_pos,
                        const float* rnd_size, const float* rnd_offx, const float* rnd_offy, int count,
                        int H, int W, int frame_h, int frame_w, int size, int kind, float macro, int n_imgs,
                        float* tables);

typedef struct aph_vit aph_vit;
typedef struct {
  int32_t patch;
  int32_t width;
  int32_t layers;
  int32_t heads;
  int32_t out_dim;
  int32_t res;
  int32_t max_batch;
  int32_t reserved;
} aph_vit_config;
int aph_vit_create(aph_vit** vit, const aph_vit_config* cfg);
int aph_vit_destroy(aph_vit* vit);
int aph_vit_load_tensor(aph_vit* vit, const char* key, const float* data, int64_t numel, void* stream);
int aph_vit_finalize(aph_vit* vit);
int aph_vit_fwd(aph_vit* vit, const float* images, int S, float* emb, int save_for_bwd, void* stream);
int aph_vit_patch_operand(aph_vit* vit, int S, void** patches_bf16, int* patch, int* grid);
int aph_vit_fwd_prepatched(aph_vit* vit, int S, float* emb, int save_for_bwd, void* stream);
int aph_vit_bwd(aph_vit* vit, const float* grad_emb, int S, float* grad_images, void* stream);
int64_t aph_vit_bytes(const aph_vit* vit);

typedef struct aph_text aph_text;
typedef struct {
  int32_t width;
  int32_t layers;
  int32_t heads;
  int32_t out_dim;
  int32_t context;
  int32_t vocab;
  int32_t max_batch;
  int32_t reserved;
} aph_text_config;
int aph_text_create(aph_text** t, const aph_text_config* cfg);
int aph_text_destroy(aph_text* t);
int aph_text_load_tensor(aph_text* t, const char* key, const float* data, int64_t numel, void* stream);
int aph_text_finalize(aph_text* t);
int aph_text_fwd(aph_text* t, const int64_t* tokens, int n, float* emb, void* stream);
int64_t aph_text_bytes(const aph_text* t);

int aph_gemm_bf16_tn(const void* A, const void* B, float* C, int M, int N, int K, void* stream);

int aph_gemm_epi_test(const void* A, const void* B, int M, int N, int K, const float* bias, const float* resid,
                      const void* gelu_in, int act, float* out_f32, void* out_bf16, void* out_pre,
                      int unpatch_p, int unpatch_g, void* stream);
int64_t aph_gemm_variant_launches(int variant, int epi);

int aph_prof_gemm(int enable, double* total_ms, double* total_flops, int* launches);

int aph_sim_fwd(const float* v1, int n1, const float* v2, int S, int D, int kind,
                float* value, float* grad_v1, float* grad_v2, void* stream);

int aph_derivat_fwd(const float* img, int C, int H, int W, double* sums, float* value, void* stream);
int aph_derivat_bwd(const float* img, int C, int H, int W, const float* upstream, float* grad_img, void* stream);
int aph_head_fwd(const float* emb, int S, int D, const float* w, const float* b, float* out, void* stream);
int aph_head_bwd(const float* grad_out, const float* w, int S, int D, float* grad_emb, void* stream);

int aph_adam_step(float* p, const float* g, float* m, float* v, int64_t n,
                  float lr, float b1, float b2, float eps, int step, void* stream);

int aph_synth_fft_bwd_adam(aph_fft_plan* plan, const float* grad_out, const float* out, const float* x_raw,
                           double* stats, const float* scale, float contrast, const float* colmat_host,
                           int apply_sigmoid, float* grad_params, float* params, float* m, float* v,
                           float lr, float b1, float b2, float eps, int step, void* stream);

int aph_allreduce_sym(uint64_t mc_ptr, const uint64_t* peer_ptrs, const uint64_t* signal_pads_dev, int rank, int world,
                      int64_t numel, int* err_flag, void* stream);

int64_t aph_launch_count(void);

#ifdef __cplusplus
}
#endif
#endif
```

Before: 100.3.

## Restrict last ViT layer's post-attention work to CLS rows via strided GEMMs

In the final transformer layer only the CLS token feeds the output, so the out-projection, LN2, MLP and their backward GEMMs now run on S rows instead of S*T, using new row-stride support (lda, ld_out, ld_resid) in the TMA GEMM path. Backward seeds the last layer's gradient into a compact CLS buffer and folds it back into the full-token gradient inside the LN1 backward kernel, removing two full memsets. This adds a zero-initialised sparse attention-gradient buffer and stride plumbing, and the strided A/tensor-map loads may be less efficient.

```diff
diff --git a/aphantasia_b200/_lib.py b/aphantasia_b200/_lib.py
--- a/aphantasia_b200/_lib.py
+++ b/aphantasia_b200/_lib.py
@@ -51,6 +51,8 @@
     'aph_gemm_bf16_tn': (C.c_int, [C.c_void_p, C.c_void_p, c_f32p, C.c_int, C.c_int, C.c_int, C.c_void_p]),
     'aph_gemm_epi_test': (C.c_int, [C.c_void_p, C.c_void_p, C.c_int, C.c_int, C.c_int, c_f32p, c_f32p, C.c_void_p, C.c_int, c_f32p, C.c_void_p, C.c_void_p,
                                     C.c_int, C.c_int, C.c_void_p]),
+    'aph_gemm_epi_strided_test': (C.c_int, [C.c_void_p, C.c_int, C.c_void_p, C.c_int, C.c_int, C.c_int, c_f32p, c_f32p, C.c_int, C.c_void_p,
+                                            C.c_int, c_f32p, C.c_void_p, C.c_void_p, C.c_int, C.c_void_p]),
     'aph_gemm_variant_launches': (C.c_int64, [C.c_int, C.c_int]),
     'aph_prof_gemm': (C.c_int, [C.c_int, C.POINTER(C.c_double), C.POINTER(C.c_double), C.POINTER(C.c_int)]),
     'aph_sim_fwd': (C.c_int, [c_f32p, C.c_int, c_f32p, C.c_int, C.c_int, C.c_int, c_f32p, c_f32p, c_f32p, C.c_void_p]),
diff --git a/aphantasia_b200/csrc/tc_gemm.cuh b/aphantasia_b200/csrc/tc_gemm.cuh
--- a/aphantasia_b200/csrc/tc_gemm.cuh
+++ b/aphantasia_b200/csrc/tc_gemm.cuh
@@ -16,6 +16,8 @@
   int act = 0;
   int unpatch_p = 0;
   int unpatch_g = 0;
+  int ld_resid = 0;
+  int ld_out = 0;
 };
 
 struct GemmShape { int M, N, K; };
@@ -158,12 +160,13 @@
 constexpr bool epi_bf16_out() { return EPI == EPI_BF16 || EPI == EPI_BIAS_BF16 || EPI == EPI_BIAS_GELU || EPI == EPI_GELUGRAD_BF16; }
 
 template <int EPI>
-__device__ __forceinline__ void epi_store2(const GemmEpi& epi, int N, int row, int col, float v0, float v1, float2 bb) {
-  const size_t off = (size_t)row * N + col;
+__device__ __forceinline__ void epi_store2(const GemmEpi& epi, size_t out_row, size_t res_row, int row, int col, float v0, float v1,
+                                           float2 bb) {
+  const size_t off = out_row + col;
   if (EPI == EPI_F32) {
     *reinterpret_cast<float2*>(epi.out_f32 + off) = make_float2(v0, v1);
   } else if (EPI == EPI_BIAS_RESID) {
-    const float2 r = __ldg(reinterpret_cast<const float2*>(epi.resid + off));
+    const float2 r = __ldg(reinterpret_cast<const float2*>(epi.resid + res_row + col));
     *reinterpret_cast<float2*>(epi.out_f32 + off) = make_float2(v0 + bb.x + r.x, v1 + bb.y + r.y);
   } else {
     const int p = epi.unpatch_p, g = epi.unpatch_g, R = p * g;
@@ -192,9 +195,9 @@
 }
 
 template <int EPI>
-__device__ __forceinline__ void epi_store_bf16x32(const GemmEpi& epi, int N, int row, bool valid, int col0, int q, const float* v,
+__device__ __forceinline__ void epi_store_bf16x32(const GemmEpi& epi, int row, bool valid, int col0, int q, const float* v,
                                                   const float2* bb) {
-  const size_t off = (size_t)row * N + col0 + 8 * q;
+  const size_t off = (size_t)row * epi.ld_out + col0 + 8 * q;
   uint32_t w[4], w2[4];
   if constexpr (EPI == EPI_GELUGRAD_BF16) {
     uint4 g = make_uint4(0u, 0u, 0u, 0u);
@@ -316,16 +319,18 @@
               v0[2 * t] = d[h][4 * (j0 + t)]; v0[2 * t + 1] = d[h][4 * (j0 + t) + 1];
               v1[2 * t] = d[h][4 * (j0 + t) + 2]; v1[2 * t + 1] = d[h][4 * (j0 + t) + 3];
             }
-            epi_store_bf16x32<EPI>(epi, shp.N, row0, row0 < shp.M, col0, lane & 3, v0, bb);
-            epi_store_bf16x32<EPI>(epi, shp.N, row1, row1 < shp.M, col0, lane & 3, v1, bb);
+            epi_store_bf16x32<EPI>(epi, row0, row0 < shp.M, col0, lane & 3, v0, bb);
+            epi_store_bf16x32<EPI>(epi, row1, row1 < shp.M, col0, lane & 3, v1, bb);
           }
         } else {
+          const size_t out0 = (size_t)row0 * epi.ld_out, out1 = out0 + 8 * (size_t)epi.ld_out;
+          const size_t res0 = (EPI == EPI_BIAS_RESID) ? (size_t)row0 * epi.ld_resid : 0, res1 = res0 + 8 * (size_t)epi.ld_resid;
 #pragma unroll
           for (int j = 0; j < BN / 8; ++j) {
             const int col = n_blk * BN + 8 * j + col_in_tile;
             const float2 bb = HAS_BIAS ? __ldg(reinterpret_cast<const float2*>(epi.bias + col)) : make_float2(0.f, 0.f);
-            if (row0 < shp.M) epi_store2<EPI>(epi, shp.N, row0, col, d[h][4 * j], d[h][4 * j + 1], bb);
-            if (row1 < shp.M) epi_store2<EPI>(epi, shp.N, row1, col, d[h][4 * j + 2], d[h][4 * j + 3], bb);
+            if (row0 < shp.M) epi_store2<EPI>(epi, out0, res0, row0, col, d[h][4 * j], d[h][4 * j + 1], bb);
+            if (row1 < shp.M) epi_store2<EPI>(epi, out1, res1, row1, col, d[h][4 * j + 2], d[h][4 * j + 3], bb);
           }
         }
       }
@@ -333,8 +338,8 @@
   }
 }
 
-int make_tmap_bf16(CUtensorMap* out, const void* base, int rows, int K, int box_rows);
+int make_tmap_bf16(CUtensorMap* out, const void* base, int rows, int K, int box_rows, int64_t row_stride = 0);
 int make_tmap_bf16_tokens(CUtensorMap* out, const void* base, int cols, int T, int S, int box_rows);
-int launch_gemm(const void* A, const void* B, GemmShape shp, const GemmEpi& epi, cudaStream_t st);
-
-}
+int launch_gemm(const void* A, const void* B, GemmShape shp, const GemmEpi& epi, cudaStream_t st, int lda = 0);
+
+}
diff --git a/aphantasia_b200/csrc/vit.cu b/aphantasia_b200/csrc/vit.cu
--- a/aphantasia_b200/csrc/vit.cu
+++ b/aphantasia_b200/csrc/vit.cu
@@ -42,11 +42,14 @@
   float* emb_int = nullptr;
   bf16* d_emb = nullptr;
   float* d_cls = nullptr;
+  float* dxc = nullptr;
+  bf16* dxc_bf = nullptr;
   float* dx = nullptr;
   bf16* dx_bf = nullptr;
   bf16* dh = nullptr;
   bf16* d_ln = nullptr;
   bf16* d_attn = nullptr;
+  bf16* d_attn_last = nullptr;
   bf16* d_qkv = nullptr;
   bf16* d_tok = nullptr;
   int last_S = -1;
@@ -56,6 +59,11 @@
   unsigned long long stamp = 0;
   int graph_misses = 0;
 };
+
+static size_t stat_off(const VitImpl* v, int k) {
+  const size_t Mmax = (size_t)v->cfg.max_batch * v->T, k2 = 2 * (size_t)v->cfg.layers;
+  return (size_t)k < k2 ? k * Mmax : k2 * Mmax + (k - k2) * (size_t)v->cfg.max_batch;
+}
 
 bool gemm_profiling_on();
 
@@ -184,17 +192,21 @@
     e |= dev_alloc(v, &l.w_proj, (size_t)4 * D * D); e |= dev_alloc(v, &l.w_proj_t, (size_t)4 * D * D);
   }
   e |= dev_alloc(v, &v->patches, Mp * v->Kp); e |= dev_alloc(v, &v->tok, Mp * D); e |= dev_alloc(v, &v->e, M * D);
-  v->xs.resize(2 * Ly + 1); for (auto& x : v->xs) e |= dev_alloc(v, &x, M * D);
+  v->xs.resize(2 * Ly + 1);
+  for (int i = 0; i <= 2 * Ly; ++i) e |= dev_alloc(v, &v->xs[i], (i >= 2 * Ly - 1 ? (size_t)S : M) * D);
   e |= dev_alloc(v, &v->ln_out, M * D); e |= dev_alloc(v, &v->attn_out, M * D); e |= dev_alloc(v, &v->h_act, M * 4 * D);
   v->qkv.resize(Ly); v->h_pre.resize(Ly);
-  for (int i = 0; i < Ly; ++i) { e |= dev_alloc(v, &v->qkv[i], M * 3 * D); e |= dev_alloc(v, &v->h_pre[i], M * 4 * D); }
-  e |= dev_alloc(v, &v->st_mean, (size_t)(2 * Ly + 2) * M); e |= dev_alloc(v, &v->st_rstd, (size_t)(2 * Ly + 2) * M);
+  for (int i = 0; i < Ly; ++i) { e |= dev_alloc(v, &v->qkv[i], M * 3 * D); e |= dev_alloc(v, &v->h_pre[i], (i == Ly - 1 ? (size_t)S : M) * 4 * D); }
+  e |= dev_alloc(v, &v->st_mean, stat_off(v, 2 * Ly + 2)); e |= dev_alloc(v, &v->st_rstd, stat_off(v, 2 * Ly + 2));
   e |= dev_alloc(v, &v->cls_ln, (size_t)S * D); e |= dev_alloc(v, &v->emb_int, (size_t)S * O);
   e |= dev_alloc(v, &v->d_emb, (size_t)S * O); e |= dev_alloc(v, &v->d_cls, (size_t)S * D);
+  e |= dev_alloc(v, &v->dxc, (size_t)S * D); e |= dev_alloc(v, &v->dxc_bf, (size_t)S * D);
   e |= dev_alloc(v, &v->dx, M * D); e |= dev_alloc(v, &v->dx_bf, M * D); e |= dev_alloc(v, &v->dh, M * 4 * D);
-  e |= dev_alloc(v, &v->d_ln, M * D); e |= dev_alloc(v, &v->d_attn, M * D); e |= dev_alloc(v, &v->d_qkv, M * 3 * D);
-  e |= dev_alloc(v, &v->d_tok, Mp * D);
+  e |= dev_alloc(v, &v->d_ln, M * D); e |= dev_alloc(v, &v->d_attn, M * D); e |= dev_alloc(v, &v->d_attn_last, M * D);
+  e |= dev_alloc(v, &v->d_qkv, M * 3 * D); e |= dev_alloc(v, &v->d_tok, Mp * D);
   if (e) { aph_vit_destroy(reinterpret_cast<aph_vit*>(v)); return 1; }
+  APH_CUDA_OK(cudaMemset(v->d_attn_last, 0, M * D * sizeof(bf16)));
+  APH_CUDA_OK(cudaDeviceSynchronize());
   APH_CUDA_OK(cudaFuncSetAttribute(k_attn_fwd, cudaFuncAttributeMaxDynamicSharedMemorySize, (int)attn_fwd_smem(T)));
   APH_CUDA_OK(cudaFuncSetAttribute(k_attn_bwd, cudaFuncAttributeMaxDynamicSharedMemorySize, (int)attn_bwd_smem(T)));
   *out = reinterpret_cast<aph_vit*>(v);
@@ -307,7 +319,6 @@
   const int rc = run_cached(v->fwd_graphs, v->warm_fwd, v->stamp, v->graph_misses, nullptr, nullptr, S, save_for_bwd, st, [&]() -> int {
   const int D = v->D, T = v->T, g = v->g, Ly = v->cfg.layers, O = v->cfg.out_dim, H = v->cfg.heads;
   const int M = S * T, Mp = S * g * g;
-  const size_t Mmax = (size_t)v->cfg.max_batch * T;
   int e;
   {
     GemmEpi ep; ep.out_f32 = v->tok;
@@ -318,27 +329,29 @@
   }
   for (int l = 0; l < Ly; ++l) {
     const LayerW& w = v->L[l];
+    const bool last = l == Ly - 1;
+    const int Mr = last ? S : M, ld_tok = last ? T * D : 0;
     float* x_in = v->xs[2 * l]; float* x_mid = v->xs[2 * l + 1]; float* x_out = v->xs[2 * l + 2];
-    float* mean1 = v->st_mean + (size_t)(1 + 2 * l) * Mmax; float* rstd1 = v->st_rstd + (size_t)(1 + 2 * l) * Mmax;
-    float* mean2 = mean1 + Mmax; float* rstd2 = rstd1 + Mmax;
+    float* mean1 = v->st_mean + stat_off(v, 1 + 2 * l); float* rstd1 = v->st_rstd + stat_off(v, 1 + 2 * l);
+    float* mean2 = v->st_mean + stat_off(v, 2 + 2 * l); float* rstd2 = v->st_rstd + stat_off(v, 2 + 2 * l);
     NCH_DISPATCH(D, APH_CUDA_OK(launch_k(k_ln_fwd<NCH>, dim3(rows_grid(M)), dim3(256), (size_t)0, st, 1, x_in, (size_t)D, w.ln1_w, w.ln1_b, v->ln_out, mean1, rstd1, M, D)));
     APH_LAUNCH_OK();
     { GemmEpi ep; ep.bias = w.b_qkv; ep.out_bf16 = v->qkv[l];
       if ((e = launch_gemm(v->ln_out, w.w_qkv, GemmShape{M, 3 * D, D}, ep, st))) return e; }
     if (attn_simt()) { k_attn_fwd<<<S * H, 256, attn_fwd_smem(T), st>>>(v->qkv[l], v->attn_out, T, D, H); APH_LAUNCH_OK(); }
     else if ((e = attn_dispatch(true, v->qkv[l], nullptr, v->attn_out, S, T, D, H, st))) return e;
-    { GemmEpi ep; ep.bias = w.b_o; ep.resid = x_in; ep.out_f32 = x_mid;
-      if ((e = launch_gemm(v->attn_out, w.w_o, GemmShape{M, D, D}, ep, st))) return e; }
-    NCH_DISPATCH(D, APH_CUDA_OK(launch_k(k_ln_fwd<NCH>, dim3(rows_grid(M)), dim3(256), (size_t)0, st, 1, x_mid, (size_t)D, w.ln2_w, w.ln2_b, v->ln_out, mean2, rstd2, M, D)));
+    { GemmEpi ep; ep.bias = w.b_o; ep.resid = x_in; ep.ld_resid = ld_tok; ep.out_f32 = x_mid;
+      if ((e = launch_gemm(v->attn_out, w.w_o, GemmShape{Mr, D, D}, ep, st, ld_tok))) return e; }
+    NCH_DISPATCH(D, APH_CUDA_OK(launch_k(k_ln_fwd<NCH>, dim3(rows_grid(Mr)), dim3(256), (size_t)0, st, 1, x_mid, (size_t)D, w.ln2_w, w.ln2_b, v->ln_out, mean2, rstd2, Mr, D)));
     APH_LAUNCH_OK();
     { GemmEpi ep; ep.bias = w.b_fc; ep.out_pre = v->h_pre[l]; ep.act = 1; ep.out_bf16 = v->h_act;
-      if ((e = launch_gemm(v->ln_out, w.w_fc, GemmShape{M, 4 * D, D}, ep, st))) return e; }
+      if ((e = launch_gemm(v->ln_out, w.w_fc, GemmShape{Mr, 4 * D, D}, ep, st))) return e; }
     { GemmEpi ep; ep.bias = w.b_proj; ep.resid = x_mid; ep.out_f32 = x_out;
-      if ((e = launch_gemm(v->h_act, w.w_proj, GemmShape{M, D, 4 * D}, ep, st))) return e; }
+      if ((e = launch_gemm(v->h_act, w.w_proj, GemmShape{Mr, D, 4 * D}, ep, st))) return e; }
   }
   {
-    float* meanp = v->st_mean + (size_t)(2 * Ly + 1) * Mmax; float* rstdp = v->st_rstd + (size_t)(2 * Ly + 1) * Mmax;
-    NCH_DISPATCH(D, APH_CUDA_OK(launch_k(k_ln_fwd<NCH>, dim3(rows_grid(S)), dim3(256), (size_t)0, st, 1, v->xs[2 * Ly], (size_t)T * D, v->lnpost_w, v->lnpost_b, v->cls_ln,
+    float* meanp = v->st_mean + stat_off(v, 2 * Ly + 1); float* rstdp = v->st_rstd + stat_off(v, 2 * Ly + 1);
+    NCH_DISPATCH(D, APH_CUDA_OK(launch_k(k_ln_fwd<NCH>, dim3(rows_grid(S)), dim3(256), (size_t)0, st, 1, v->xs[2 * Ly], (size_t)D, v->lnpost_w, v->lnpost_b, v->cls_ln,
                                                                  meanp, rstdp, S, D)));
     APH_LAUNCH_OK();
     GemmEpi ep; ep.out_f32 = v->emb_int;
@@ -365,39 +378,42 @@
   const int rc = run_cached(v->bwd_graphs, v->warm_bwd, v->stamp, v->graph_misses, nullptr, nullptr, S, 0, st, [&]() -> int {
   const int D = v->D, T = v->T, Ly = v->cfg.layers, O = v->cfg.out_dim, H = v->cfg.heads;
   const int M = S * T;
-  const size_t Mmax = (size_t)v->cfg.max_batch * T;
   int e;
   {
     GemmEpi ep; ep.out_f32 = v->d_cls;
     if ((e = launch_gemm(v->d_emb, v->w_out_t, GemmShape{S, D, O}, ep, st))) return e;
-    APH_CUDA_OK(cudaMemsetAsync(v->dx, 0, (size_t)M * D * sizeof(float), st));
-    APH_CUDA_OK(cudaMemsetAsync(v->dx_bf, 0, (size_t)M * D * sizeof(bf16), st));
-    float* meanp = v->st_mean + (size_t)(2 * Ly + 1) * Mmax; float* rstdp = v->st_rstd + (size_t)(2 * Ly + 1) * Mmax;
-    NCH_DISPATCH(D, APH_CUDA_OK(launch_k(k_ln_bwd<NCH>, dim3(rows_grid(S)), dim3(256), (size_t)0, st, 1, v->d_cls, v->xs[2 * Ly], meanp, rstdp, v->lnpost_w, v->dx, v->dx_bf,
-                                                                 S, T, D, 1, 0)));
+    float* meanp = v->st_mean + stat_off(v, 2 * Ly + 1); float* rstdp = v->st_rstd + stat_off(v, 2 * Ly + 1);
+    NCH_DISPATCH(D, APH_CUDA_OK(launch_k(k_ln_bwd<NCH>, dim3(rows_grid(S)), dim3(256), (size_t)0, st, 1, v->d_cls, v->xs[2 * Ly], meanp, rstdp, v->lnpost_w, v->dxc, v->dxc_bf,
+                                                                 S, T, D, 0, 0, (const float*)nullptr)));
     APH_LAUNCH_OK();
   }
   for (int l = Ly - 1; l >= 0; --l) {
     const LayerW& w = v->L[l];
+    const bool last = l == Ly - 1;
+    const int Mr = last ? S : M;
+    float* gx = last ? v->dxc : v->dx; bf16* gx_bf = last ? v->dxc_bf : v->dx_bf; bf16* d_attn = last ? v->d_attn_last : v->d_attn;
     float* x_in = v->xs[2 * l]; float* x_mid = v->xs[2 * l + 1];
-    float* mean1 = v->st_mean + (size_t)(1 + 2 * l) * Mmax; float* rstd1 = v->st_rstd + (size_t)(1 + 2 * l) * Mmax;
-    float* mean2 = mean1 + Mmax; float* rstd2 = rstd1 + Mmax;
+    float* mean1 = v->st_mean + stat_off(v, 1 + 2 * l); float* rstd1 = v->st_rstd + stat_off(v, 1 + 2 * l);
+    float* mean2 = v->st_mean + stat_off(v, 2 + 2 * l); float* rstd2 = v->st_rstd + stat_off(v, 2 + 2 * l);
     { GemmEpi ep; ep.gelu_in = v->h_pre[l]; ep.out_bf16 = v->dh;
-      if ((e = launch_gemm(v->dx_bf, w.w_proj_t, GemmShape{M, 4 * D, D}, ep, st))) return e; }
+      if ((e = launch_gemm(gx_bf, w.w_proj_t, GemmShape{Mr, 4 * D, D}, ep, st))) return e; }
     { GemmEpi ep; ep.out_bf16 = v->d_ln;
-      if ((e = launch_gemm(v->dh, w.w_fc_t, GemmShape{M, D, 4 * D}, ep, st))) return e; }
-    NCH_DISPATCH(D, APH_CUDA_OK(launch_k(k_ln_bwd<NCH, bf16>, dim3(rows_grid(M)), dim3(256), (size_t)0, st, 1, v->d_ln, x_mid, mean2, rstd2, w.ln2_w, v->dx, v->dx_bf, M, T, D, 0, 1)));
-    APH_LAUNCH_OK();
-    { GemmEpi ep; ep.out_bf16 = v->d_attn;
-      if ((e = launch_gemm(v->dx_bf, w.w_o_t, GemmShape{M, D, D}, ep, st))) return e; }
-    if (attn_simt()) { k_attn_bwd<<<S * H, 256, attn_bwd_smem(T), st>>>(v->qkv[l], v->d_attn, v->d_qkv, T, D, H); APH_LAUNCH_OK(); }
-    else if ((e = attn_dispatch(false, v->qkv[l], v->d_attn, v->d_qkv, S, T, D, H, st))) return e;
+      if ((e = launch_gemm(v->dh, w.w_fc_t, GemmShape{Mr, D, 4 * D}, ep, st))) return e; }
+    NCH_DISPATCH(D, APH_CUDA_OK(launch_k(k_ln_bwd<NCH, bf16>, dim3(rows_grid(Mr)), dim3(256), (size_t)0, st, 1, v->d_ln, x_mid, mean2, rstd2, w.ln2_w, gx, gx_bf, Mr, T, D, 0, 1,
+                                         (const float*)nullptr)));
+    APH_LAUNCH_OK();
+    { GemmEpi ep; ep.out_bf16 = d_attn; ep.ld_out = last ? T * D : 0;
+      if ((e = launch_gemm(gx_bf, w.w_o_t, GemmShape{Mr, D, D}, ep, st))) return e; }
+    if (attn_simt()) { k_attn_bwd<<<S * H, 256, attn_bwd_smem(T), st>>>(v->qkv[l], d_attn, v->d_qkv, T, D, H); APH_LAUNCH_OK(); }
+    else if ((e = attn_dispatch(false, v->qkv[l], d_attn, v->d_qkv, S, T, D, H, st))) return e;
     { GemmEpi ep; ep.out_bf16 = v->d_ln;
       if ((e = launch_gemm(v->d_qkv, w.w_qkv_t, GemmShape{M, D, 3 * D}, ep, st))) return e; }
-    NCH_DISPATCH(D, APH_CUDA_OK(launch_k(k_ln_bwd<NCH, bf16>, dim3(rows_grid(M)), dim3(256), (size_t)0, st, 1, v->d_ln, x_in, mean1, rstd1, w.ln1_w, v->dx, v->dx_bf, M, T, D, 0, 1)));
-    APH_LAUNCH_OK();
-  }
-  NCH_DISPATCH(D, APH_CUDA_OK(launch_k(k_ln_bwd<NCH>, dim3(rows_grid(M)), dim3(256), (size_t)0, st, 1, v->dx, v->e, v->st_mean, v->st_rstd, v->lnpre_w, nullptr, v->d_tok, M, T, D, 2, 0)));
+    NCH_DISPATCH(D, APH_CUDA_OK(launch_k(k_ln_bwd<NCH, bf16>, dim3(rows_grid(M)), dim3(256), (size_t)0, st, 1, v->d_ln, x_in, mean1, rstd1, w.ln1_w, v->dx, v->dx_bf, M, T, D,
+                                         last ? 1 : 0, 1, (const float*)(last ? v->dxc : nullptr))));
+    APH_LAUNCH_OK();
+  }
+  NCH_DISPATCH(D, APH_CUDA_OK(launch_k(k_ln_bwd<NCH>, dim3(rows_grid(M)), dim3(256), (size_t)0, st, 1, v->dx, v->e, v->st_mean, v->st_rstd, v->lnpre_w, nullptr, v->d_tok, M, T, D, 2, 0,
+                                       (const float*)nullptr)));
   APH_LAUNCH_OK();
   return 0;
   });
diff --git a/aphantasia_b200/csrc/vit_gemm.cu b/aphantasia_b200/csrc/vit_gemm.cu
--- a/aphantasia_b200/csrc/vit_gemm.cu
+++ b/aphantasia_b200/csrc/vit_gemm.cu
@@ -22,12 +22,14 @@
   return fn;
 }
 
-int make_tmap_bf16(CUtensorMap* out, const void* base, int rows, int K, int box_rows) {
+int make_tmap_bf16(CUtensorMap* out, const void* base, int rows, int K, int box_rows, int64_t row_stride) {
   EncodeTiledFn enc = get_encode();
   APH_REQUIRE(enc != nullptr, "cuTensorMapEncodeTiled not available from the driver");
-  APH_REQUIRE((reinterpret_cast<uintptr_t>(base) & 15) == 0 && K % 8 == 0, "tensor map: base/stride not 16-byte aligned");
+  if (row_stride == 0) row_stride = K;
+  APH_REQUIRE(row_stride >= K, "tensor map: row stride %lld < K=%d", (long long)row_stride, K);
+  APH_REQUIRE((reinterpret_cast<uintptr_t>(base) & 15) == 0 && row_stride % 8 == 0, "tensor map: base/stride not 16-byte aligned");
   const cuuint64_t gdim[2] = {(cuuint64_t)K, (cuuint64_t)rows};
-  const cuuint64_t gstride[1] = {(cuuint64_t)K * 2};
+  const cuuint64_t gstride[1] = {(cuuint64_t)row_stride * 2};
   const cuuint32_t box[2] = {(cuuint32_t)GEMM_BK, (cuuint32_t)box_rows};
   const cuuint32_t estr[2] = {1, 1};
   const CUresult r = enc(out, CU_TENSOR_MAP_DATA_TYPE_BFLOAT16, 2, const_cast<void*>(base), gdim, gstride, box, estr,
@@ -60,7 +62,7 @@
 static std::atomic<long long> g_variant_launches[2][EPI_KINDS];
 
 template <int BN, bool PINGPONG, int EPI>
-static int launch_cfg(const void* A, const void* B, GemmShape shp, const GemmEpi& epi, cudaStream_t st) {
+static int launch_cfg(const void* A, const void* B, GemmShape shp, const GemmEpi& epi, cudaStream_t st, int lda) {
   using L = GemmCfg<BN>;
   static_assert(L::SMEM <= 227 * 1024, "GEMM shared-memory budget");
   g_variant_launches[(PINGPONG || BN == 256) ? 1 : 0][EPI].fetch_add(1, std::memory_order_relaxed);
@@ -70,7 +72,7 @@
     configured = true;
   }
   CUtensorMap ma, mb;
-  if (int e = make_tmap_bf16(&ma, A, shp.M, shp.K, GEMM_BM)) return e;
+  if (int e = make_tmap_bf16(&ma, A, shp.M, shp.K, GEMM_BM, lda)) return e;
   if (int e = make_tmap_bf16(&mb, B, shp.N, shp.K, BN)) return e;
   const int tiles = ((shp.M + GEMM_BM - 1) / GEMM_BM) * (shp.N / BN);
   const int grid = tiles < num_sms() ? tiles : num_sms();
@@ -82,12 +84,19 @@
   return 0;
 }
 
-int launch_gemm(const void* A, const void* B, GemmShape shp, const GemmEpi& epi, cudaStream_t st) {
+int launch_gemm(const void* A, const void* B, GemmShape shp, const GemmEpi& epi_in, cudaStream_t st, int lda) {
   APH_REQUIRE(A && B && shp.M > 0, "gemm: null operand or empty M");
   APH_REQUIRE(shp.K % GEMM_BK == 0 && shp.K > 0, "gemm: K=%d must be a positive multiple of %d", shp.K, GEMM_BK);
   APH_REQUIRE(shp.N % 128 == 0 && shp.N > 0, "gemm: N=%d must be a positive multiple of 128", shp.N);
+  APH_REQUIRE(lda == 0 || lda >= shp.K, "gemm: lda=%d < K=%d", lda, shp.K);
+  APH_REQUIRE((epi_in.ld_out == 0 || epi_in.ld_out >= shp.N) && (epi_in.ld_resid == 0 || epi_in.ld_resid >= shp.N),
+              "gemm: output / residual row stride below N=%d", shp.N);
+  GemmEpi epi = epi_in;
+  if (epi.ld_out == 0) epi.ld_out = shp.N;
+  if (epi.ld_resid == 0) epi.ld_resid = shp.N;
   int kind = -1;
   const bool b = epi.bias, r = epi.resid, gi = epi.gelu_in, f = epi.out_f32, h = epi.out_bf16, pre = epi.out_pre, act = epi.act == 1, un = epi.unpatch_p > 0;
+  APH_REQUIRE(!un || epi.ld_out == shp.N, "gemm: the un-patchify store takes no output stride");
   if (un && f && !b && !r && !gi && !h && !pre && !act) kind = EPI_UNPATCH;
   else if (f && !h && !b && !r && !gi && !pre && !act) kind = EPI_F32;
   else if (h && !f && !b && !r && !gi && !pre && !act) kind = EPI_BF16;
@@ -97,12 +106,14 @@
   else if (h && !f && !b && !r && gi && !pre && !act) kind = EPI_GELUGRAD_BF16;
   APH_REQUIRE(kind >= 0, "gemm: unsupported epilogue combination");
   const uintptr_t bf16_ptrs = reinterpret_cast<uintptr_t>(epi.out_bf16) | reinterpret_cast<uintptr_t>(epi.out_pre) | reinterpret_cast<uintptr_t>(epi.gelu_in);
-  APH_REQUIRE((bf16_ptrs & 15) == 0, "gemm: bf16 epilogue operands must be 16-byte aligned (8 columns are stored per lane)");
+  APH_REQUIRE((bf16_ptrs & 15) == 0 && ((size_t)epi.ld_out * (f ? 4 : 2)) % 16 == 0 && ((size_t)epi.ld_resid * 4) % 16 == 0 &&
+              ((size_t)lda * 2) % 16 == 0,
+              "gemm: bf16 epilogue operands and row strides must be 16-byte aligned (8 columns are stored per lane)");
   const int m_tiles = (shp.M + GEMM_BM - 1) / GEMM_BM;
   const bool pingpong = m_tiles * (shp.N / 128) >= 2 * num_sms() && shp.K <= 1024;
   const bool wide = !pingpong && shp.N % 256 == 0 && m_tiles * (shp.N / 256) >= num_sms();
-#define APH_GEMM_CASE(K) case K: return pingpong ? launch_cfg<128, true, K>(A, B, shp, epi, st) \
-                                                 : wide ? launch_cfg<256, false, K>(A, B, shp, epi, st) : launch_cfg<128, false, K>(A, B, shp, epi, st);
+#define APH_GEMM_CASE(K) case K: return pingpong ? launch_cfg<128, true, K>(A, B, shp, epi, st, lda) \
+                                                 : wide ? launch_cfg<256, false, K>(A, B, shp, epi, st, lda) : launch_cfg<128, false, K>(A, B, shp, epi, st, lda);
   switch (kind) {
     APH_GEMM_CASE(EPI_F32) APH_GEMM_CASE(EPI_BF16) APH_GEMM_CASE(EPI_BIAS_BF16) APH_GEMM_CASE(EPI_BIAS_GELU)
     APH_GEMM_CASE(EPI_BIAS_RESID) APH_GEMM_CASE(EPI_GELUGRAD_BF16) APH_GEMM_CASE(EPI_UNPATCH)
@@ -132,6 +143,16 @@
   return launch_gemm(A, B, GemmShape{M, N, K}, epi, (cudaStream_t)stream);
 }
 
+extern "C" int aph_gemm_epi_strided_test(const void* A, int lda, const void* B, int M, int N, int K, const float* bias,
+                                         const float* resid, int ld_resid, const void* gelu_in, int act, float* out_f32,
+                                         void* out_bf16, void* out_pre, int ld_out, void* stream) {
+  GemmEpi epi;
+  epi.bias = bias; epi.resid = resid; epi.gelu_in = reinterpret_cast<const bf16*>(gelu_in); epi.act = act;
+  epi.out_f32 = out_f32; epi.out_bf16 = reinterpret_cast<bf16*>(out_bf16); epi.out_pre = reinterpret_cast<bf16*>(out_pre);
+  epi.ld_resid = ld_resid; epi.ld_out = ld_out;
+  return launch_gemm(A, B, GemmShape{M, N, K}, epi, (cudaStream_t)stream, lda);
+}
+
 extern "C" int64_t aph_gemm_variant_launches(int variant, int epi) {
   if (variant < 0 || variant > 1 || epi >= EPI_KINDS) return -1;
   long long n = 0;
diff --git a/aphantasia_b200/csrc/vit_ops.cuh b/aphantasia_b200/csrc/vit_ops.cuh
--- a/aphantasia_b200/csrc/vit_ops.cuh
+++ b/aphantasia_b200/csrc/vit_ops.cuh
@@ -152,29 +152,28 @@
 __global__ void __launch_bounds__(256) k_ln_bwd(const DY* __restrict__ dy, const float* __restrict__ x, const float* __restrict__ mean,
                                                 const float* __restrict__ rstd, const float* __restrict__ gamma,
                                                 float* __restrict__ dx, bf16* __restrict__ dx_bf16, int rows, int T, int D,
-                                                int mode, int accumulate) {
+                                                int mode, int accumulate, const float* __restrict__ dcls) {
   pdl_trigger(); pdl_wait();
   const int r = (blockIdx.x * blockDim.x + threadIdx.x) >> 5, lane = threadIdx.x & 31;
   if (r >= rows) return;
   constexpr int N = 4 * NCH;
-  const size_t row = (mode == 1) ? (size_t)r * T : (size_t)r;
+  const size_t row = (size_t)r;
   if (mode == 2 && (r % T) == 0) return;
   float v[N], xv[N], gm[N];
-  load_row(dy + (size_t)r * D, v, lane);
+  load_row(dy + row * D, v, lane);
   load_row(x + row * D, xv, lane);
   load_row(gamma, gm, lane);
-  const int sidx = (mode == 1) ? r : (int)row;
-  ln_bwd_row(v, xv, gm, mean[sidx], rstd[sidx], D);
+  ln_bwd_row(v, xv, gm, mean[row], rstd[row], D);
   if (mode == 2) {
     const int s = r / T, t = r - s * T;
     store_row_bf16(dx_bf16 + ((size_t)s * (T - 1) + (t - 1)) * D, v, lane);
     return;
   }
-  if (accumulate) {
+  if (mode == 1 ? (r % T) == 0 : accumulate != 0) {
     float a[N];
-    load_row(dx + row * D, a, lane);
-    #pragma unroll
-  for (int i = 0; i < N; ++i) v[i] += a[i];
+    load_row(mode == 1 ? dcls + (size_t)(r / T) * D : dx + row * D, a, lane);
+    #pragma unroll
+    for (int i = 0; i < N; ++i) v[i] += a[i];
   }
   store_row_f32(dx + row * D, v, lane);
   store_row_bf16(dx_bf16 + row * D, v, lane);
diff --git a/include/aphb200.h b/include/aphb200.h
--- a/include/aphb200.h
+++ b/include/aphb200.h
@@ -128,6 +128,9 @@
 int aph_gemm_epi_test(const void* A, const void* B, int M, int N, int K, const float* bias, const float* resid,
                       const void* gelu_in, int act, float* out_f32, void* out_bf16, void* out_pre,
                       int unpatch_p, int unpatch_g, void* stream);
+int aph_gemm_epi_strided_test(const void* A, int lda, const void* B, int M, int N, int K, const float* bias,
+                              const float* resid, int ld_resid, const void* gelu_in, int act, float* out_f32,
+                              void* out_bf16, void* out_pre, int ld_out, void* stream);
 int64_t aph_gemm_variant_launches(int variant, int epi);
 
 int aph_prof_gemm(int enable, double* total_ms, double* total_flops, int* launches);
```

Result: faster. 104.4 (median of 6 runs) (+4.1%).
